# CamilleChallier/Contrastive-Masked-UNet

Hardware: AMD Instinct MI355X
Metric: pretrain images/sec/node at 512x512 (CM-UNet masked-reconstruction step) (higher is better)
Workload: dtype f16; 1 GPU; cmunet_masked_recon_unet64x5_512x512_bs32_mask0.6; optimizer=AdamW(fused), amp=dynamic loss scale (device-side GradScaler protocol), global_batch=32, parallelism=dp1

## Files before the change

### cmunet_amd/_lib.py

```python
import ctypes
import os
import subprocess

_HERE = os.path.dirname(os.path.abspath(__file__))
CSRC = os.path.join(_HERE, "csrc")
LIB_PATH = os.environ.get("CMU_LIB_PATH") or os.path.join(CSRC, "libcmunet_hip.so")

F32, F16, BF16 = 0, 1, 2

_P = ctypes.c_void_p
_I = ctypes.c_int
_L = ctypes.c_int64
_F = ctypes.c_float
_U64 = ctypes.c_uint64
_D = ctypes.c_double

_SIGS = {
    "cmu_last_error": (ctypes.c_char_p, []),
    "cmu_last_kernel": (ctypes.c_char_p, []),
    "cmu_softmax2_threshold": (_I, [_P, _F, _P, _I, _I, _I, _P]),
    "cmu_conv3x3_c1_wgrad_bn": (_I, [_P, _P, _I, _P, _L, _P, _L, _P, _P, _P, _P, _P, _P, _I, _I, _I, _I, _I, _P, _P]),
    "cmu_conv3x3_c1_wgrad_bn_w": (_I, [_P, _P, _I, _P, _L, _P, _P, _P, _P, _P, _P, _P, _I, _I, _I, _I, _I, _P, _P]),
    "cmu_soft_skeleton_ws_bytes": (_L, [_L]),
    "cmu_soft_skeleton": (_I, [_P, _P, _I, _I, _I, _I, _P, _P]),
# ... 37 lines not shown
    "cmu_dtype_size": (_I, [_I]),
    "cmu_pack_conv3x3_elems": (_L, [_I, _I, _I, _I]),
    "cmu_pack_conv3x3": (_I, [_P, _P, _I, _I, _I, _I, _P]),
    "cmu_pack_convT2x2_elems": (_L, [_I, _I, _I, _I]),
    "cmu_pack_convT2x2": (_I, [_P, _P, _I, _I, _I, _I, _P]),
    "cmu_conv3x3_c1_fwd": (_I, [_P, _P, _I, _P, _P, _L, _P, _I, _I, _I, _I, _I, _P]),
    "cmu_conv3x3_fwd": (_I, [_P, _L, _P, _P, _I, _P, _P, _L, _P, _I, _I, _I, _I, _I, _I, _P]),
    "cmu_conv_ntiles": (_I, [_I, _I, _I]),
    "cmu_bn_finalize_ws_bytes": (_L, [_I]),
    "cmu_bn_finalize": (_I, [_P, _I, _L, _P, _P, _P, _P, _P, _F, _F, _I, _P, _P, _P, _P, _I, _P, _P]),
    "cmu_bnrelu_maxpool_fwd": (_I, [_P, _L, _P, _P, _P, _L, _I, _I, _I, _I, _I, _P]),
    "cmu_convT2x2_fwd": (_I, [_P, _L, _P, _P, _I, _P, _P, _P, _L, _I, _I, _I, _I, _I, _I, _P]),
    "cmu_conv1x1_head_fwd": (_I, [_P, _L, _P, _P, _P, _P, _P, _I, _I, _I, _I, _I, _I, _P]),
    "cmu_apply_to_nchw": (_I, [_P, _L, _P, _P, _I, _P, _I, _I, _I, _I, _I, _P]),
    "cmu_nchw_to_nhwc": (_I, [_P, _P, _L, _I, _I, _I, _I, _I, _P]),
    "cmu_nhwc_to_nchw": (_I, [_P, _L, _P, _I, _I, _I, _I, _I, _P]),
    "cmu_bn_bwd_ws_bytes": (_L, [_I]),
    "cmu_bn_bwd_reduce": (_I, [_P, _L, _P, _L, _P, _P, _P, _P, _P, _P, _P, _I, _I, _I, _I, _I, _P, _P]),
    "cmu_bn_bwd_apply": (_I, [_P, _L, _P, _L, _P, _P, _P, _P, _P, _P, _L, _I, _I, _I, _I, _I, _P]),
    "cmu_conv3x3_wgrad_ws_bytes": (_L, [_I, _I, _I, _I, _I, _I]),
    "cmu_conv3x3_wgrad": (_I, [_P, _L, _P, _P, _I, _P, _L, _P, _I, _I, _I, _I, _I, _I, _P, _P]),
    "cmu_conv3x3_c1_wgrad_ws_bytes": (_L, [_I, _I, _I, _I]),
    "cmu_conv3x3_c1_wgrad": (_I, [_P, _P, _I, _P, _L, _P, _I, _I, _I, _I, _I, _P, _P]),
    "cmu_maxpool_bwd": (_I, [_P, _L, _P, _L, _P, _L, _P, _P, _P, _L, _P, _P, _P, _I, _I, _I, _I, _I, _P]),
    "cmu_maxpool_bwd2": (_I, [_P, _L, _P, _L, _P, _L, _P, _L, _P, _P, _P, _L, _P, _P, _P, _I, _I, _I, _I, _I, _P]),
    "cmu_maxpool_bwd_apply": (_I, [_P, _L, _P, _L, _P, _L, _P, _L, _P, _P, _P, _P, _P, _P, _L, _I, _I, _I, _I, _I, _P]),
    "cmu_bnrelu_maxpool_fwd_masked": (_I, [_P, _L, _P, _P, _P, _I, _P, _L, _I, _I, _I, _I, _I, _P]),
    "cmu_maxpool_bwd_masked": (_I, [_P, _L, _P, _L, _P, _L, _P, _P, _P, _I, _P, _L, _I, _I, _I, _I, _I, _P]),
    "cmu_bn_bwd_finalize": (_I, [_P, _L, _P, _P, _P, _I, _P]),
    "cmu_convT2x2_dgrad": (_I, [_P, _L, _P, _P, _L, _I, _I, _I, _I, _I, _I, _P]),
    "cmu_convT2x2_dgrad_bn": (_I, [_P, _L, _P, _P, _L, _P, _L, _P, _P, _P, _P, _P, _I, _I, _I, _I, _I, _I, _P]),
    "cmu_conv3x3_dgrad_bn": (_I, [_P, _L, _P, _P, _L, _P, _L, _P, _P, _P, _P, _P, _I, _I, _I, _I, _I, _I, _P]),
    "cmu_bn_bwd_finalize_tiles": (_I, [_P, _I, _L, _P, _P, _P, _I, _P, _P]),
    "cmu_convT2x2_wgrad_ws_bytes": (_L, [_I, _I, _I, _I, _I, _I]),
    "cmu_convT2x2_wgrad": (_I, [_P, _L, _P, _P, _I, _P, _L, _P, _P, _I, _I, _I, _I, _I, _I, _P, _P]),
    "cmu_conv1x1_head_bwd_ws_bytes": (_L, [_I, _I, _I, _I, _I]),
    "cmu_conv1x1_head_bn_apply": (_I, [_P, _P, _L, _P, _P, _P, _P, _P, _P, _P, _L, _I, _I, _I, _I, _I, _I, _P]),
    "cmu_conv1x1_head_bwd": (_I, [_P, _P, _L, _P, _P, _P, _P, _L, _P, _P, _P, _P, _P, _I, _I, _I, _I, _I, _I, _P, _P]),
    "cmu_masked_mse_ws_bytes": (_L, [_I, _I]),
    "cmu_masked_mse_fwd_bwd": (_I, [_P, _I, _I, _P, _P, _P, _P, _F, _P, _I, _I, _I, _P, _P]),
    "cmu_softmax_ce_dice_ws_bytes": (_L, [_I, _I, _I]),
    "cmu_softmax_ce_dice_fwd_bwd": (_I, [_P, _P, _P, _P, _F, _I, _I, _I, _P, _P]),
    "cmu_infonce_inbatch_fwd_bwd": (_I, [_P, _P, _P, _P, _I, _I, _I, _I, _F, _F, _P]),
    "cmu_moco_ws_bytes": (_L, [_I, _I, _I]),
    "cmu_moco_infonce_enqueue": (_I, [_P, _P, _P, _I, _P, _P, _P, _P, _P, _I, _I, _I, _F, _P, _P]),
    "cmu_l2_normalize_rows": (_I, [_P, _P, _I, _I, _P]),
    "cmu_l2_normalize_rows_bwd": (_I, [_P, _P, _P, _I, _I, _P]),
    "cmu_moco_logits_assemble": (_I, [_P, _P, _P, _P, _I, _I, _I, _F, _P]),
    "cmu_moco_logits_split": (_I, [_P, _P, _I, _I, _F, _P]),
    "cmu_moco_logits_addpos": (_I, [_P, _P, _P, _I, _I, _I, _F, _P]),
    "cmu_row_cross_entropy": (_I, [_P, _P, _P, _P, _P, _P, _I, _I, _P]),
    "cmu_scale_by_device_scalar": (_I, [_P, _P, _L, _P]),
    "cmu_patchify": (_I, [_P, _P, _I, _I, _I, _I, _I, _I, _P]),
    "cmu_masked_stats_rows": (_I, []),
    "cmu_masked_channel_stats": (_I, [_P, _L, _P, _I, _I, _P, _I, _I, _I, _I, _I, _P]),
    "cmu_mask_select": (_I, [_P, _L, _P, _P, _I, _P, _I, _I, _P, _P, _L, _I, _I, _I, _I, _I, _P]),
    "cmu_bn_bwd_reduce_masked": (_I, [_P, _L, _P, _L, _P, _P, _P, _P, _P, _P, _P, _P, _I, _L, _I, _I, _I, _I, _I, _P, _P]),
    "cmu_bn_bwd_apply_masked": (_I, [_P, _L, _P, _L, _P, _P, _P, _P, _P, _P, _L, _P, _I, _I, _I, _I, _I, _I, _P]),
    "cmu_sparse_tile_list": (_I, [_P, _I, _I, _I, _I, _I, _I, _P, _P, _P]),
    "cmu_conv3x3_tiles_supported": (_I, [_I, _I, _I, _I, _I, _I]),
    "cmu_rows_channel_stats": (_I, [_P, _L, _P, _P, _P, _I, _I, _I, _I, _I, _P]),
    "cmu_bn_bwd_reduce_rows": (_I, [_P, _L, _P, _L, _P, _P, _P, _P, _P, _P, _P, _P, _P, _L, _L, _I, _I, _I, _I, _I, _P, _P]),
    "cmu_sparse_tile_lists_max": (_I, []),
    "cmu_sparse_tile_lists": (_I, [_P, _I, _I, _I, _P, _P, _P, _P, _P, _P]),
    "cmu_sparse_pixel_lists": (_I, [_P, _P, _I, _I, _I, _P, _P, _P, _P, _P]),
    "cmu_conv3x3_c1_fwd_tiles_rows": (_I, [_L]),
# ... 191 lines not shown
```

### cmunet_amd/csrc/backward_elem.hip

```cpp
#include "common.h"

constexpr int RED_MAX_BLOCKS = 2048;
#ifndef CMU_POOLB_BLOCKS
#define CMU_POOLB_BLOCKS 2048
#endif
#ifndef CMU_HEADB_BLOCKS
#define CMU_HEADB_BLOCKS 768
#endif
#ifndef CMU_POOLA_PPT
#define CMU_POOLA_PPT 0
#endif
constexpr int POOLB_MAX_BLOCKS = CMU_POOLB_BLOCKS, HEADB_MAX_BLOCKS = CMU_HEADB_BLOCKS;
constexpr int BNWS_HDR = 16;

__device__ static inline float sum_over_rows(float v, float* red, int tid, int cpb, int ppb) {
    __syncthreads();
    red[tid] = v;
    __syncthreads();
    float a = 0.f;
    if (tid < cpb)
        for (int k = 0; k < ppb; ++k) a += red[k * cpb + tid];
    return a;
}

constexpr int FOLD_G = 8;
template <int NV>
__device__ static inline void fold_rows(float (&v)[NV], float* red, int tid, int cpb, int ppb) {
    const int lane = tid & 63, wv = tid >> 6;
    if (cpb <= 64) {
#pragma unroll
        for (int i = 0; i < NV; ++i)
            for (int o = cpb; o < 64; o <<= 1) v[i] += __shfl_xor(v[i], o, 64);
    }
#pragma unroll
    for (int g0 = 0; g0 < NV; g0 += FOLD_G) {
        __syncthreads();
        if (cpb <= 64) {
            if (lane < cpb) {
#pragma unroll
                for (int i = g0; i < g0 + FOLD_G && i < NV; ++i) red[((i - g0) * 4 + wv) * 64 + lane] = v[i];
            }
        } else {
#pragma unroll
            for (int i = g0; i < g0 + FOLD_G && i < NV; ++i) red[(i - g0) * 256 + tid] = v[i];
        }
        __syncthreads();
// ... 66 lines not shown
#pragma unroll
        for (int e = 0; e < EPC; ++e) { t[e] = s1[e]; t[EPC + e] = s2[e]; }
        fold_rows<2 * EPC>(t, red, tid, cpb, ppb);
        if (tid < cpb && blockIdx.y * cpb + tid < nchunk) {
#pragma unroll
            for (int e = 0; e < EPC; ++e) {
                const int c = (blockIdx.y * cpb + tid) * EPC + e;
                ws[((int64_t)blockIdx.x * 2 + 0) * C + c] = t[e];
                ws[((int64_t)blockIdx.x * 2 + 1) * C + c] = t[EPC + e];
            }
        }
        return;
    }
#pragma unroll
    for (int e = 0; e < EPC; ++e) {
        const float a = sum_over_rows(s1[e], red, tid, cpb, ppb);
        const float b = sum_over_rows(s2[e], red, tid, cpb, ppb);
        if (tid < cpb && blockIdx.y * cpb + tid < nchunk) {
            const int c = (blockIdx.y * cpb + tid) * EPC + e;
            ws[((int64_t)blockIdx.x * 2 + 0) * C + c] = a;
            ws[((int64_t)blockIdx.x * 2 + 1) * C + c] = b;
        }
    }
}

__global__ __launch_bounds__(256) void bn_bwd_final_kernel(const float* __restrict__ ws, double count, float* dgamma,
                                                          float* dbeta, float* coef, int C) {
    __shared__ double red[2][16][16];
    const int nblocks = *reinterpret_cast<const int*>(ws);
    ws += BNWS_HDR / 4;
    const int cl = threadIdx.x & 15, part = threadIdx.x >> 4;
    const int c = blockIdx.x * 16 + cl;
    double s1 = 0.0, s2 = 0.0;
    if (c < C) {
        constexpr int U = 8;
        int b = part;
        for (; b + 16 * (U - 1) < nblocks; b += 16 * U) {
            float a[U], q[U];
#pragma unroll
            for (int u = 0; u < U; ++u) {
                a[u] = ws[((int64_t)(b + 16 * u) * 2 + 0) * C + c];
                q[u] = ws[((int64_t)(b + 16 * u) * 2 + 1) * C + c];
            }
#pragma unroll
            for (int u = 0; u < U; ++u) {
                s1 += (double)a[u];
                s2 += (double)q[u];
            }
        }
        for (; b < nblocks; b += 16) {
            s1 += (double)ws[((int64_t)b * 2 + 0) * C + c];
            s2 += (double)ws[((int64_t)b * 2 + 1) * C + c];
        }
    }
    red[0][part][cl] = s1;
    red[1][part][cl] = s2;
    __syncthreads();
    if (part != 0 || c >= C) return;
    s1 = 0.0; s2 = 0.0;
    for (int q = 0; q < 16; ++q) { s1 += red[0][q][cl]; s2 += red[1][q][cl]; }
    if (dbeta) dbeta[c] = (float)s1;
    if (dgamma) dgamma[c] = (float)s2;
    coef[c] = (float)(s1 / count);
    coef[C + c] = (float)(s2 / count);
}

static void chunk_geometry(int nchunk, int* cpb, int* ppb, int* gy) {
    *cpb = nchunk < 256 ? nchunk : 256;
    *ppb = 256 / *cpb;
    *gy = cmu_div_up(nchunk, *cpb);
}

template <class TR>
static int bn_bwd_reduce_t(const void* dA, int64_t ldd, const void* y, int64_t ldy, const float* scale, const float* shift,
                           const float* mean, const float* invstd, float* dgamma, float* dbeta, float* coef, int B, int H, int W,
                           int C, void* ws, const uint8_t* active, int f, int64_t count, hipStream_t st, const int* rows = nullptr,
                           const int* n_rows = nullptr, int64_t max_rows = 0) {
    int cpb, ppb, gy;
    chunk_geometry(C / TR::EPC, &cpb, &ppb, &gy);
    const int64_t npix = (int64_t)B * H * W;
    const int sbits = active ? sp_shift_bits(H, f) : 0;
    const int64_t nloop = rows ? max_rows : npix;
    int gx = (int)(cmu_div_up64(nloop, ppb * 4) < RED_MAX_BLOCKS ? cmu_div_up64(nloop, ppb * 4) : RED_MAX_BLOCKS);
    if (gx < 1) gx = 1;
    hipLaunchKernelGGL((bn_bwd_reduce_kernel<TR>), dim3(gx, gy), dim3(256), 0, st, (const unsigned char*)dA, ldd,
                       (const unsigned char*)y, ldy, scale, shift, mean, invstd, (float*)ws, npix, C, cpb, ppb, active, f, sbits, H, W, rows,
                       n_rows);
// ... 141 lines not shown
}
extern "C" int cmu_bn_bwd_apply(const void* dA, int64_t ldd, const void* y, int64_t ldy, const float* scale, const float* shift,
                                const float* save_mean, const float* save_invstd, const float* coef, void* dY, int64_t ldo, int B,
                                int H, int W, int C, int dt, void* stream) {
    int rc;
    if ((rc = check_pair("cmu_bn_bwd_apply", dA, ldd, y, ldy, C, dt))) return rc;
    if ((rc = check_pair("cmu_bn_bwd_apply(dY)", dY, ldo, y, ldy, C, dt))) return rc;
    CMU_CHECK_ARG(scale && shift && save_mean && save_invstd && coef && B > 0 && H > 0 && W > 0, "cmu_bn_bwd_apply: null argument");
    CMU_DISPATCH_DT(dt, bn_bwd_apply_t, dA, ldd, y, ldy, scale, shift, save_mean, save_invstd, coef, dY, ldo, B, H, W, C,
                    (const uint8_t*)nullptr, 0, (hipStream_t)stream);
}
extern "C" int cmu_bn_bwd_apply_masked(const void* dA, int64_t ldd, const void* y, int64_t ldy, const float* scale, const float* shift,
                                       const float* save_mean, const float* save_invstd, const float* coef, void* dY, int64_t ldo,
                                       const uint8_t* active, int f, int B, int H, int W, int C, int dt, void* stream) {
    int rc;
    if ((rc = check_pair("cmu_bn_bwd_apply_masked", dA, ldd, y, ldy, C, dt))) return rc;
    if ((rc = check_pair("cmu_bn_bwd_apply_masked(dY)", dY, ldo, y, ldy, C, dt))) return rc;
    CMU_CHECK_ARG(scale && shift && save_mean && save_invstd && coef && active && B > 0, "cmu_bn_bwd_apply_masked: null argument");
    CMU_CHECK_ARG(sp_shift_bits(H, f) >= 0 && (f << sp_shift_bits(H, f)) == W, "cmu_bn_bwd_apply_masked: H,W must be f times a power of two");
    CMU_DISPATCH_DT(dt, bn_bwd_apply_t, dA, ldd, y, ldy, scale, shift, save_mean, save_invstd, coef, dY, ldo, B, H, W, C, active, f,
                    (hipStream_t)stream);
}

template <class TR, int MODE>
__global__ __launch_bounds__(256) void maxpool_bwd_kernel(const unsigned char* __restrict__ dP, int64_t ldp,
                                                         const unsigned char* __restrict__ dS, int64_t lds,
                                                         const unsigned char* __restrict__ dS2, int64_t lds2,
                                                         const unsigned char* __restrict__ y, int64_t ldy,
                                                         const float* __restrict__ scale, const float* __restrict__ shift,
                                                         unsigned char* __restrict__ dA, int64_t lda, int B, int H, int W, int C,
                                                         int cpb, int ppb, const float* __restrict__ mean,
                                                         const float* __restrict__ invstd, float* __restrict__ bn_ws,
                                                         const float* __restrict__ coef, const uint8_t* __restrict__ amask = nullptr,
                                                         int mf = 0, int msbits = 0) {
    constexpr int EPC = TR::EPC;
    constexpr int ES = (int)sizeof(typename TR::elem_t);
    __shared__ float red[MODE == 2 ? 1 : FOLD_G * 256];
    const int tid = threadIdx.x;
    const int nchunk = C / EPC;
    const int ch = blockIdx.y * cpb + tid % cpb;
    const int prow = tid / cpb;
    const bool active = prow < ppb && ch < nchunk;
    const int Ho = H / 2, Wo = W / 2;
    const int64_t npool = (int64_t)B * Ho * Wo;
    float sc[EPC], sh[EPC], mu[EPC], is[EPC], s1[EPC], s2[EPC], c1[EPC], c2[EPC];
#pragma unroll
    for (int e = 0; e < EPC; ++e) {
        const int c = active ? ch * EPC + e : 0;
        sc[e] = scale[c];
        sh[e] = shift[c];
        mu[e] = (bn_ws || MODE == 2) ? mean[c] : 0.f;
        is[e] = (bn_ws || MODE == 2) ? invstd[c] : 0.f;
        c1[e] = MODE == 2 ? coef[c] : 0.f;
        c2[e] = MODE == 2 ? coef[C + c] : 0.f;
        s1[e] = s2[e] = 0.f;
    }
    constexpr int PPT = (MODE == 2 && CMU_POOLA_PPT > 0) ? CMU_POOLA_PPT : 0;
    const int64_t span = PPT > 0 ? (int64_t)ppb * PPT : (int64_t)gridDim.x * ppb;
    if (active)
        for (int64_t rng = (int64_t)blockIdx.x * (PPT > 0 ? span : ppb); rng < npool; rng += (PPT > 0 ? (int64_t)gridDim.x * span : npool))
        for (int64_t pp = rng + prow; pp < npool && (PPT == 0 || pp < rng + span); pp += (PPT > 0 ? ppb : span)) {
            int xo, yo, b;
            cmu_pixel_coords(pp, Wo, Ho, npool <= 0x7fffffffll, b, yo, xo);
            if (amask != nullptr && !sp_active(amask, mf, msbits, b, 2 * yo, 2 * xo, 0)) continue;
            float best[EPC], g[EPC], f[4][EPC];
            int arg[EPC];
            TR::unpack(ld_global16_nt(dP + (pp * ldp + ch * EPC) * ES), g);
            int64_t src[4];
#pragma unroll
            for (int q = 0; q < 4; ++q) {
                src[q] = ((int64_t)b * H + 2 * yo + (q >> 1)) * W + 2 * xo + (q & 1);
                TR::unpack(ld_global16(y + (src[q] * ldy + ch * EPC) * ES), f[q]);
#pragma unroll
                for (int e = 0; e < EPC; ++e) {
                    const float a = fmaxf(fmaf(f[q][e], sc[e], sh[e]), 0.f);
// ... 42 lines not shown
        }
    if (MODE == 2 || bn_ws == nullptr) return;
    if (blockIdx.x == 0 && blockIdx.y == 0 && tid == 0) *reinterpret_cast<int*>(bn_ws) = (int)gridDim.x;
    float* ws = bn_ws + BNWS_HDR / 4;
    if (fold_ok(cpb)) {
        float t[2 * EPC];
#pragma unroll
        for (int e = 0; e < EPC; ++e) { t[e] = s1[e]; t[EPC + e] = s2[e]; }
        fold_rows<2 * EPC>(t, red, tid, cpb, ppb);
        if (tid < cpb && blockIdx.y * cpb + tid < nchunk) {
#pragma unroll
            for (int e = 0; e < EPC; ++e) {
                const int c = (blockIdx.y * cpb + tid) * EPC + e;
                ws[((int64_t)blockIdx.x * 2 + 0) * C + c] = t[e];
                ws[((int64_t)blockIdx.x * 2 + 1) * C + c] = t[EPC + e];
            }
        }
        return;
    }
#pragma unroll
    for (int e = 0; e < EPC; ++e) {
        const float a = sum_over_rows(s1[e], red, tid, cpb, ppb);
        const float bsum = sum_over_rows(s2[e], red, tid, cpb, ppb);
        if (tid < cpb && blockIdx.y * cpb + tid < nchunk) {
            const int c = (blockIdx.y * cpb + tid) * EPC + e;
            ws[((int64_t)blockIdx.x * 2 + 0) * C + c] = a;
            ws[((int64_t)blockIdx.x * 2 + 1) * C + c] = bsum;
        }
    }
}
template <class TR>
static int maxpool_bwd_t(const void* dP, int64_t ldp, const void* dS, int64_t lds, const void* dS2, int64_t lds2, const void* y, int64_t ldy, const float* scale,
                         const float* shift, void* dA, int64_t lda, int B, int H, int W, int C, const float* mean, const float* invstd,
                         void* bn_ws, hipStream_t st, const float* coef = nullptr, const uint8_t* amask = nullptr, int mf = 0) {
    int cpb, ppb, gy;
    chunk_geometry(C / TR::EPC, &cpb, &ppb, &gy);
    const int64_t npool = (int64_t)B * (H / 2) * (W / 2);
    int gx = (int)(cmu_div_up64(npool, ppb * 2) < POOLB_MAX_BLOCKS ? cmu_div_up64(npool, ppb * 2) : POOLB_MAX_BLOCKS);
    if (coef != nullptr && CMU_POOLA_PPT > 0) {
        const int64_t nb = cmu_div_up64(npool, (int64_t)ppb * (CMU_POOLA_PPT > 0 ? CMU_POOLA_PPT : 1));
        gx = (int)(nb < (1 << 20) ? nb : (1 << 20));
    }
    if (gx < 1) gx = 1;
#define CMU_POOLB_LAUNCH(MODE_)                                                                                                            \
    hipLaunchKernelGGL((maxpool_bwd_kernel<TR, MODE_>), dim3(gx, gy), dim3(256), 0, st, (const unsigned char*)dP, ldp, (const unsigned char*)dS, lds, \
                       (const unsigned char*)dS2, lds2, (const unsigned char*)y, ldy, scale, shift, (unsigned char*)dA, lda, B, H, W, C, cpb, ppb, \
                       mean, invstd, (float*)bn_ws, coef, amask, mf, amask ? sp_shift_bits(H, mf) : 0)
    if (coef != nullptr) CMU_POOLB_LAUNCH(2);
    else if (dA == nullptr) CMU_POOLB_LAUNCH(1);
    else CMU_POOLB_LAUNCH(0);
#undef CMU_POOLB_LAUNCH
    CMU_CHECK_LAUNCH("cmu_maxpool_bwd");
    return CMU_OK;
}
extern "C" int cmu_maxpool_bwd2(const void* dP, int64_t ldp, const void* dSkip, int64_t lds, const void* dSkip2, int64_t lds2, const void* y,
                                int64_t ldy, const float* scale, const float* shift, void* dA, int64_t lda, const float* save_mean,
                                const float* save_invstd, void* bn_ws, int B, int H, int W, int C, int dt, void* stream) {
    CMU_CHECK_ARG(bn_ws == nullptr || (save_mean && save_invstd), "cmu_maxpool_bwd: fused BN statistics need save_mean / save_invstd");
    CMU_CHECK_ARG(dSkip2 == nullptr || dSkip != nullptr, "cmu_maxpool_bwd2: dSkip2 without dSkip");
    int rc;
    if ((rc = check_pair("cmu_maxpool_bwd(dP,y)", dP, ldp, y, ldy, C, dt))) return rc;
    CMU_CHECK_ARG(dA != nullptr || bn_ws != nullptr, "cmu_maxpool_bwd: dA may only be NULL in the statistics-only form (bn_ws given)");
    if (dA && (rc = check_pair("cmu_maxpool_bwd(dA,y)", dA, lda, y, ldy, C, dt))) return rc;
    if (dSkip && (rc = check_pair("cmu_maxpool_bwd(dSkip,y)", dSkip, lds, y, ldy, C, dt))) return rc;
    if (dSkip2 && (rc = check_pair("cmu_maxpool_bwd2(dSkip2,y)", dSkip2, lds2, y, ldy, C, dt))) return rc;
    CMU_CHECK_ARG(scale && shift && B > 0 && H > 0 && W > 0 && H % 2 == 0 && W % 2 == 0, "cmu_maxpool_bwd: bad dims (%d,%d)", H, W);
    CMU_DISPATCH_DT(dt, maxpool_bwd_t, dP, ldp, dSkip, lds, dSkip2, lds2, y, ldy, scale, shift, dA, lda, B, H, W, C, save_mean, save_invstd,
                    bn_ws, (hipStream_t)stream);
}
extern "C" int cmu_maxpool_bwd_masked(const void* dP, int64_t ldp, const void* dSkip, int64_t lds, const void* y, int64_t ldy, const float* scale,
                                      const float* shift, const uint8_t* active, int f, void* dA, int64_t lda, int B, int H, int W, int C, int dt,
                                      void* stream) {
    CMU_CHECK_ARG(active && f > 0 && dA && scale && shift, "cmu_maxpool_bwd_masked: null argument");
    int rc;
    if ((rc = check_pair("cmu_maxpool_bwd_masked(dP,y)", dP, ldp, y, ldy, C, dt))) return rc;
    if ((rc = check_pair("cmu_maxpool_bwd_masked(dA,y)", dA, lda, y, ldy, C, dt))) return rc;
    if (dSkip && (rc = check_pair("cmu_maxpool_bwd_masked(dSkip,y)", dSkip, lds, y, ldy, C, dt))) return rc;
    CMU_CHECK_ARG(B > 0 && H > 0 && W > 0 && H % 2 == 0 && W % 2 == 0, "cmu_maxpool_bwd_masked: bad dims (%d,%d)", H, W);
    const int sbits = sp_shift_bits(H, f);
    CMU_CHECK_ARG(sbits >= 1 && (f << sbits) == W, "cmu_maxpool_bwd_masked: H=%d, W=%d must be f=%d times a power of two >= 2", H, W, f);
// ... 500 lines not shown
                  "cmu_conv3x3_c1_wgrad_bn: alignment / stride");
    CMU_DISPATCH_DT(dt, conv3x3_c1_wgrad_t, x, mask, mask_per_sample, dA, ldd, dW, B, H, W, Cout, ws, (hipStream_t)stream, yraw, ldy, scale,
                    shift, save_mean, save_invstd, coef);
}
extern "C" int cmu_conv3x3_c1_wgrad_bn_tiles(const float* x, const uint8_t* mask, int mask_per_sample, const void* dA, int64_t ldd,
                                             const void* yraw, int64_t ldy, const float* w, const float* scale, const float* shift,
                                             const float* save_mean, const float* save_invstd, const float* coef, const int* tile_list,
                                             const int* tile_count, int64_t max_tiles, float* dW, int B, int H, int W, int Cout, int dt,
                                             void* ws, void* stream) {
    const int es = cmu_dtype_size(dt);
    CMU_CHECK_ARG(es > 0 && x && dA && scale && shift && save_mean && save_invstd && coef && dW && ws && tile_list && tile_count && B > 0 && H > 0 &&
                      W > 0 && ((yraw != nullptr) != (w != nullptr)),
                  "cmu_conv3x3_c1_wgrad_bn_tiles: bad args (exactly one of yraw / w)");
    const int epc = 16 / es;
    CMU_CHECK_ARG(Cout > 0 && Cout % epc == 0 && Cout / epc <= 256, "cmu_conv3x3_c1_wgrad_bn_tiles: Cout=%d unsupported", Cout);
    CMU_CHECK_ARG(cmu_aligned16(dA) && ldd % epc == 0 && ldd >= Cout && (yraw == nullptr || (cmu_aligned16(yraw) && ldy % epc == 0 && ldy >= Cout)),
                  "cmu_conv3x3_c1_wgrad_bn_tiles: alignment / stride");
    CMU_DISPATCH_DT(dt, conv3x3_c1_wgrad_t, x, mask, mask_per_sample, dA, ldd, dW, B, H, W, Cout, ws, (hipStream_t)stream, yraw, ldy, scale, shift,
                    save_mean, save_invstd, coef, w, tile_list, tile_count, max_tiles);
}
extern "C" int cmu_conv3x3_c1_wgrad_bn_w(const float* x, const uint8_t* mask, int mask_per_sample, const void* dA, int64_t ldd,
                                         const float* w, const float* scale, const float* shift, const float* save_mean,
                                         const float* save_invstd, const float* coef, float* dW, int B, int H, int W, int Cout, int dt,
                                         void* ws, void* stream) {
    const int es = cmu_dtype_size(dt);
    CMU_CHECK_ARG(es > 0 && x && dA && w && scale && shift && save_mean && save_invstd && coef && dW && ws && B > 0 && H > 0 && W > 0,
                  "cmu_conv3x3_c1_wgrad_bn_w: bad args");
    const int epc = 16 / es;
    CMU_CHECK_ARG(Cout > 0 && Cout % epc == 0 && Cout / epc <= 256, "cmu_conv3x3_c1_wgrad_bn_w: Cout=%d unsupported", Cout);
    CMU_CHECK_ARG(cmu_aligned16(dA) && ldd % epc == 0 && ldd >= Cout, "cmu_conv3x3_c1_wgrad_bn_w: alignment / stride");
    CMU_DISPATCH_DT(dt, conv3x3_c1_wgrad_t, x, mask, mask_per_sample, dA, ldd, dW, B, H, W, Cout, ws, (hipStream_t)stream, nullptr, 0, scale,
                    shift, save_mean, save_invstd, coef, w);
}
```

### cmunet_amd/csrc/common.h

```cpp
#pragma once
#include <hip/hip_runtime.h>
#include <stdint.h>
#include <stdio.h>
#include <stdarg.h>
#include "../../include/cmunet_hip.h"

void cmu_set_error(const char* fmt, ...);
void cmu_set_kernel_tag(const char* tag);

#define CMU_CHECK_ARG(cond, ...)                 \
    do {                                         \
        if (!(cond)) {                           \
            cmu_set_error(__VA_ARGS__);          \
            return CMU_ERR_ARG;                  \
        }                                        \
    } while (0)

#define CMU_CHECK_LAUNCH(name)                                                        \
    do {                                                                              \
        hipError_t e__ = hipGetLastError();                                           \
        if (e__ != hipSuccess) {                                                      \
            cmu_set_error("%s: launch failed: %s", name, hipGetErrorString(e__));     \
            return CMU_ERR_LAUNCH;                                                    \
        }                                                                             \
// ... 179 lines not shown
        y = (int)((p / W) % H);
        b = (int)(p / ((int64_t)W * H));
    }
}

__device__ static inline bool sp_active(const uint8_t* __restrict__ active, int f, int sbits, int b, int y, int x, int invert) {
    const bool a = active[((int64_t)b * f + (y >> sbits)) * f + (x >> sbits)] != 0;
    return invert ? !a : a;
}
__host__ __device__ static inline bool cmu_relu_on(int c0, int relu_from) { return relu_from >= 0 ? c0 >= relu_from : c0 < -relu_from; }
static inline int sp_shift_bits(int H, int f) {
    int s = 0;
    while ((f << s) < H) ++s;
    return ((f << s) == H) ? s : -1;
}

constexpr int CMU_TH = 16;
constexpr int CMU_TW = 16;
__host__ __device__ static inline int cmu_div_up(int a, int b) { return (a + b - 1) / b; }
__host__ __device__ static inline int cmu_conv3x3_npad(int N) { return N <= 64 ? 64 : ((N + 127) / 128) * 128; }
static inline int64_t cmu_div_up64(int64_t a, int64_t b) { return (a + b - 1) / b; }

__device__ static inline void philox4x32_10(uint32_t c0, uint32_t c1, uint32_t c2, uint32_t c3, uint32_t k0, uint32_t k1, uint32_t* out) {
#pragma unroll
    for (int r = 0; r < 10; ++r) {
        const uint32_t hi0 = __umulhi(0xD2511F53u, c0), lo0 = 0xD2511F53u * c0;
        const uint32_t hi1 = __umulhi(0xCD9E8D57u, c2), lo1 = 0xCD9E8D57u * c2;
        const uint32_t n0 = hi1 ^ c1 ^ k0, n1 = lo1, n2 = hi0 ^ c3 ^ k1, n3 = lo0;
        c0 = n0; c1 = n1; c2 = n2; c3 = n3;
        k0 += 0x9E3779B9u; k1 += 0xBB67AE85u;
    }
    out[0] = c0; out[1] = c1; out[2] = c2; out[3] = c3;
}
```

### cmunet_amd/csrc/conv_igemm.hip

```cpp
#include "common.h"
#include <stdlib.h>

enum { MODE_CONV3 = 0, MODE_CONVT_FWD = 1, MODE_CONVT_DGRAD = 2 };

struct IGParams {
    const void* x;
    int64_t ldx;
    const float* in_scale;
    const float* in_shift;
    int relu_from;
    const void* w;
    int npad;
    void* y;
    int64_t ldy;
    float* stats;
    const float* bias;
    int B, H, W;
    int K;
    int N;
    int Cq;
    int nslices;
    int nslices32;
    int tilesX, tilesY, nblk;
    int64_t total_blocks;
    const void* bx;
    int64_t ldbx;
    const float *b_scale, *b_shift, *b_mean, *b_invstd;
    float* bstats;
    int buf_ok;
    unsigned fd_nblk[2], fd_tx[2], fd_ty[2];
    const int* tile_list;
    const int* tile_count;
};
static inline void cmu_fastdiv_init(unsigned d, unsigned* out) {
    unsigned s = 0;
    while ((1ull << s) < d) ++s;
    out[0] = (unsigned)((((1ull << s) - d) << 32) / d + 1);
    out[1] = s;
}

template <class TR, int MODE>
struct IGCfg {
    typedef typename TR::elem_t elem_t;
    static constexpr bool C3 = (MODE == MODE_CONV3);
    static constexpr int TAPS = C3 ? 9 : 2;
    static constexpr int HALO = C3 ? 1 : 0;
    static constexpr int LW = CMU_TW + 2 * HALO;
    static constexpr int LH = CMU_TH + 2 * HALO;
    static constexpr int NPIX = LW * LH;
    static constexpr int SLICES_A = C3 ? 1 : TAPS;
    static constexpr int PS_A = SLICES_A * 64 + 16;
    static constexpr int A_BYTES = NPIX * PS_A;
    static constexpr int PS_W = 80;
    static constexpr int BN = 64;
    static constexpr int W_BYTES = TAPS * BN * PS_W;
    static constexpr int KC = 64 / (int)sizeof(elem_t);
    static constexpr int EPC = TR::EPC;
    static constexpr int EPI_ROW = BN * (int)sizeof(elem_t) + 16;
    static constexpr int EPI_STAGE = 4 * 64 * EPI_ROW;
    static constexpr int EPI_BYTES = EPI_STAGE + 4 * BN * 2 * 4;
    static constexpr int MAIN_BYTES = A_BYTES + W_BYTES;
    static constexpr int LDS_BYTES = MAIN_BYTES > EPI_BYTES ? MAIN_BYTES : EPI_BYTES;
    static constexpr int A_CHUNKS = NPIX * SLICES_A * 4;
    static constexpr int A_ITERS = (A_CHUNKS + 255) / 256;
    static constexpr int W_CHUNKS = TAPS * BN * 4;
    static constexpr int W_ITERS = (W_CHUNKS + 255) / 256;
// ... 263 lines not shown
        IG_STAMP(5);
    }
    __syncthreads();

    float* stat_lds = reinterpret_cast<float*>(smem + C::EPI_STAGE);
    if (MODE == MODE_CONV3 && p.stats != nullptr) {
        float s1[2] = {0.f, 0.f}, s2[2] = {0.f, 0.f};
#pragma unroll
        for (int i = 0; i < 2; ++i)
#pragma unroll
            for (int e = 0; e < 16; ++e) {
                const int m32 = (e & 3) + 8 * (e >> 2) + 4 * h;
                const int row = 4 * wave + 2 * i + pm_row(m32), col = pm_col(m32);
                const bool ok = (ty0 + row < p.H) && (tx0 + col < p.W);
#pragma unroll
                for (int j = 0; j < 2; ++j) {
                    const float v = ok ? acc[i][j][e] : 0.f;
                    s1[j] += v;
                    s2[j] = fmaf(v, v, s2[j]);
                }
            }
#pragma unroll
        for (int j = 0; j < 2; ++j) {
            s1[j] += __shfl_xor(s1[j], 32, 64);
            s2[j] += __shfl_xor(s2[j], 32, 64);
            if (h == 0) {
                stat_lds[(wave * C::BN + 32 * j + r) * 2 + 0] = s1[j];
                stat_lds[(wave * C::BN + 32 * j + r) * 2 + 1] = s2[j];
            }
        }
    }
    constexpr int CPRp = C::BN / C::EPC;
    u32x4 xr[CPRp];
    if ((MODE != MODE_CONVT_FWD) && p.bstats != nullptr) {
#pragma unroll
        for (int it = 0; it < CPRp; ++it) {
            const int idx = it * 64 + lane;
            const int m = idx / CPRp, q = idx % CPRp;
            const int row = 4 * wave + 2 * (m >> 5) + pm_row(m & 31), col = pm_col(m & 31);
            const int gy = ty0 + row < p.H ? ty0 + row : p.H - 1, gx = tx0 + col < p.W ? tx0 + col : p.W - 1;
            int n = n0 + q * C::EPC;
            n = n < p.N ? n : 0;
            const int64_t xo = (((int64_t)b * p.H + gy) * p.W + gx) * p.ldbx + n;
            xr[it] = ld_global16(reinterpret_cast<const unsigned char*>(p.bx) + xo * (int64_t)sizeof(elem_t));
        }
    }
    unsigned char* my = smem + wave * (64 * C::EPI_ROW);
#pragma unroll
    for (int i = 0; i < 2; ++i)
#pragma unroll
        for (int j = 0; j < 2; ++j) {
            float badd = 0.f;
            if (MODE == MODE_CONVT_FWD) {
                const int n = n0 + 32 * j + r;
                if (n < p.N) badd = p.bias[n % p.Cq];
            }
#pragma unroll
            for (int e = 0; e < 16; ++e) {
                const int m = 32 * i + (e & 3) + 8 * (e >> 2) + 4 * h;
                *reinterpret_cast<elem_t*>(my + m * C::EPI_ROW + (32 * j + r) * (int)sizeof(elem_t)) =
                    TR::from_float(acc[i][j][e] + badd);
            }
        }
    __syncthreads();
    if (MODE == MODE_CONV3 && p.stats != nullptr && tid < C::BN) {
        const int n = n0 + tid;
        if (n < p.N) {
            float a = 0.f, q = 0.f;
#pragma unroll
            for (int w4 = 0; w4 < 4; ++w4) {
                a += stat_lds[(w4 * C::BN + tid) * 2 + 0];
                q += stat_lds[(w4 * C::BN + tid) * 2 + 1];
            }
            p.stats[(tile * 2 + 0) * p.N + n] = a;
            p.stats[(tile * 2 + 1) * p.N + n] = q;
        }
    }
    constexpr int CPR = C::BN / C::EPC;
    unsigned char* yb = reinterpret_cast<unsigned char*>(p.y);
    const bool bs = (MODE != MODE_CONVT_FWD) && p.bstats != nullptr;
    constexpr int EPCc = C::EPC;
    float bsc[EPCc], bsh[EPCc], bmu[EPCc], bis[EPCc], bs1[EPCc], bs2[EPCc];
    const int nq = n0 + (lane % CPR) * EPCc;
    if (bs) {
#pragma unroll
        for (int e = 0; e < EPCc; ++e) {
            const int c = nq + e < p.N ? nq + e : 0;
            bsc[e] = p.b_scale[c]; bsh[e] = p.b_shift[c]; bmu[e] = p.b_mean[c]; bis[e] = p.b_invstd[c];
            bs1[e] = bs2[e] = 0.f;
        }
    }
#pragma unroll
    for (int it = 0; it < (64 * CPR) / 64; ++it) {
        const int idx = it * 64 + lane;
        const int m = idx / CPR, q = idx % CPR;
        const int row = 4 * wave + 2 * (m >> 5) + pm_row(m & 31), col = pm_col(m & 31);
        const int gy = ty0 + row, gx = tx0 + col;
        const int n = n0 + q * C::EPC;
        if (gy < p.H && gx < p.W && n < p.N) {
            const u32x4 v = *reinterpret_cast<const u32x4*>(my + m * C::EPI_ROW + q * 16);
            int64_t off;
            if (MODE == MODE_CONVT_FWD) {
                const int ij = n / p.Cq, co = n % p.Cq;
                off = (((int64_t)b * (2 * p.H) + 2 * gy + (ij >> 1)) * (2 * p.W) + 2 * gx + (ij & 1)) * p.ldy + co;
            } else {
                off = (((int64_t)b * p.H + gy) * p.W + gx) * p.ldy + n;
            }
            st_global16(yb + off * (int64_t)sizeof(elem_t), v);
            if (bs) {
                float gv[EPCc], xv[EPCc];
                TR::unpack(v, gv);
                TR::unpack(xr[it], xv);
#pragma unroll
                for (int e = 0; e < EPCc; ++e) {
                    const float dz = fmaf(xv[e], bsc[e], bsh[e]) > 0.f ? gv[e] : 0.f;
                    bs1[e] += dz;
                    bs2[e] = fmaf(dz, xv[e], bs2[e]);
                }
            }
        }
    }
    if (bs) {
#pragma unroll
        for (int e = 0; e < EPCc; ++e) {
#pragma unroll
            for (int o = CPR; o < 64; o <<= 1) {
                bs1[e] += __shfl_xor(bs1[e], o, 64);
                bs2[e] += __shfl_xor(bs2[e], o, 64);
            }
            bs2[e] = (bs2[e] - bmu[e] * bs1[e]) * bis[e];
            if (lane < CPR) {
                stat_lds[(wave * C::BN + lane * EPCc + e) * 2 + 0] = bs1[e];
                stat_lds[(wave * C::BN + lane * EPCc + e) * 2 + 1] = bs2[e];
            }
        }
        __syncthreads();
        if (tid < C::BN && n0 + tid < p.N) {
            float a = 0.f, q = 0.f;
#pragma unroll
            for (int w4 = 0; w4 < 4; ++w4) {
                a += stat_lds[(w4 * C::BN + tid) * 2 + 0];
                q += stat_lds[(w4 * C::BN + tid) * 2 + 1];
            }
            p.bstats[(tile * 2 + 0) * p.N + n0 + tid] = a;
            p.bstats[(tile * 2 + 1) * p.N + n0 + tid] = q;
        }
    }
}

#include "conv_igemm3.inc"
#include "conv_igemm3p.inc"
#include "conv_igemm5.inc"
#include "conv_igemm6.inc"
#include "conv_gemm.inc"
#include "conv_gather.inc"

template <class TR, int MODE>
static int launch_igemm(const IGParams& p, hipStream_t st, const char* name) {
    typedef IGCfg<TR, MODE> C;
    static CmuPerDevice attr_set;
    if (!attr_set.done()) {
        hipError_t e = hipFuncSetAttribute(reinterpret_cast<const void*>(&conv_igemm_kernel<TR, MODE>),
                                           hipFuncAttributeMaxDynamicSharedMemorySize, C::LDS_BYTES);
        if (e != hipSuccess) {
            cmu_set_error("%s: hipFuncSetAttribute(%d B LDS): %s", name, C::LDS_BYTES, hipGetErrorString(e));
            return CMU_ERR_LAUNCH;
        }
        attr_set.mark();
    }
    hipLaunchKernelGGL((conv_igemm_kernel<TR, MODE>), dim3((unsigned)p.total_blocks), dim3(256), C::LDS_BYTES, st, p);
    cmu_set_kernel_tag("conv_igemm_kernel");
    CMU_CHECK_LAUNCH(name);
    return CMU_OK;
}

static int check_act(const char* name, const void* ptr, int64_t ld, int C, int dt) {
    const int epc = 16 / cmu_dtype_size(dt);
    CMU_CHECK_ARG(ptr != nullptr, "%s: null tensor", name);
// ... 343 lines not shown
    for (int i = 0; i < n; ++i) {
        const int sb = sp_shift_bits(H[i], f);
        CMU_CHECK_ARG(rows[i] && counts[i] && capacity[i] > 0 && sb >= 0 && (int64_t)B * H[i] * H[i] < (1ll << 31),
                      "cmu_sparse_pixel_lists: null list, or H must be f << s (entry %d: H=%d, f=%d)", i, H[i], f);
        q.s[i] = 1 << sb; q.H[i] = H[i]; q.rows[i] = rows[i]; q.count[i] = counts[i]; q.cap[i] = capacity[i];
        if (capacity[i] > cmax) cmax = capacity[i];
    }
    const int grid = (int)(cmu_div_up64(cmax, 256) < 4096 ? cmu_div_up64(cmax, 256) : 4096);
    hipLaunchKernelGGL(sparse_pixel_rows_multi_kernel, dim3(grid, n), dim3(256), 0, (hipStream_t)stream, patches, patch_count, q);
    CMU_CHECK_LAUNCH("cmu_sparse_pixel_lists");
    return CMU_OK;
}
extern "C" int cmu_sparse_tile_list(const uint8_t* active, int f, int B, int H, int W, int tile_h, int tile_w, int* list, int* count,
                                    void* stream) {
    CMU_CHECK_ARG(active && list && count && f > 0 && B > 0 && H > 0 && W > 0 && tile_h > 0 && tile_w > 0, "cmu_sparse_tile_list: bad args");
    const int sbits = sp_shift_bits(H, f);
    CMU_CHECK_ARG(sbits >= 0 && W == H, "cmu_sparse_tile_list: H must be f << s and the level square (H=%d, W=%d, f=%d)", H, W, f);
    const int tilesY = cmu_div_up(H, tile_h), tilesX = cmu_div_up(W, tile_w);
    CMU_CHECK_ARG((int64_t)B * tilesY * tilesX < (1ll << 30), "cmu_sparse_tile_list: too many tiles");
    hipLaunchKernelGGL(sparse_tile_list_kernel, dim3(1), dim3(1024), 0, (hipStream_t)stream, active, f, sbits, B, tilesY, tilesX, tile_h, tile_w,
                       list, count);
    CMU_CHECK_LAUNCH("cmu_sparse_tile_list");
    return CMU_OK;
}

static int check_bnstats(const char* name, const void* yraw, int64_t ldy, const float* scale, const float* shift, const float* mean,
                         const float* invstd, const float* bstats, int N, int dt) {
    int rc;
    if ((rc = check_act(name, yraw, ldy, N, dt))) return rc;
    CMU_CHECK_ARG(scale && shift && mean && invstd && bstats, "%s: null BatchNorm argument", name);
    return CMU_OK;
}

extern "C" int cmu_conv3x3_dgrad_bn(const void* dY, int64_t ldd, const void* wpacked_flip, void* dX, int64_t ldx, const void* yraw,
                                    int64_t ldy, const float* scale, const float* shift, const float* save_mean,
                                    const float* save_invstd, float* bstats, int B, int H, int W, int K, int N, int dt, void* stream) {
    CMU_CHECK_ARG(B > 0 && H > 0 && W > 0 && K > 0 && N > 0, "cmu_conv3x3_dgrad_bn: bad dims");
    CMU_CHECK_ARG(cmu_dtype_size(dt) > 0, "cmu_conv3x3_dgrad_bn: bad dtype %d", dt);
    int rc;
    if ((rc = check_act("cmu_conv3x3_dgrad_bn(dY)", dY, ldd, K, dt))) return rc;
    if ((rc = check_act("cmu_conv3x3_dgrad_bn(dX)", dX, ldx, N, dt))) return rc;
    if ((rc = check_bnstats("cmu_conv3x3_dgrad_bn(yraw)", yraw, ldy, scale, shift, save_mean, save_invstd, bstats, N, dt))) return rc;
    CMU_CHECK_ARG(wpacked_flip && cmu_aligned16(wpacked_flip), "cmu_conv3x3_dgrad_bn: packed weights null/unaligned");
    CMU_CHECK_ARG((int64_t)B * cmu_div_up(H, CMU_TH) * cmu_div_up(W, CMU_TW) * cmu_div_up(N, 64) < (1ll << 31), "cmu_conv3x3_dgrad_bn: grid too large");
    IGParams p = {};
    p.x = dY; p.ldx = ldd; p.w = wpacked_flip; p.y = dX; p.ldy = ldx;
    p.B = B; p.H = H; p.W = W; p.K = K; p.N = N; p.Cq = N;
    p.bx = yraw; p.ldbx = ldy; p.b_scale = scale; p.b_shift = shift; p.b_mean = save_mean; p.b_invstd = save_invstd; p.bstats = bstats;
    fill_tiles(p);
    CMU_DISPATCH_DT(dt, conv3x3_fwd_t, p, (hipStream_t)stream);
}

extern "C" int cmu_convT2x2_dgrad_bn(const void* dOut, int64_t ldd, const void* wpacked_dgrad, void* dX, int64_t ldx, const void* yraw,
                                     int64_t ldy, const float* scale, const float* shift, const float* save_mean,
                                     const float* save_invstd, float* bstats, int B, int H, int W, int Cin, int Cout, int dt,
                                     void* stream) {
    CMU_CHECK_ARG(B > 0 && H > 0 && W > 0 && Cin > 0 && Cout > 0, "cmu_convT2x2_dgrad_bn: bad dims");
    CMU_CHECK_ARG(cmu_dtype_size(dt) > 0, "cmu_convT2x2_dgrad_bn: bad dtype %d", dt);
    int rc;
    if ((rc = check_act("cmu_convT2x2_dgrad_bn(dOut)", dOut, ldd, Cout, dt))) return rc;
    if ((rc = check_act("cmu_convT2x2_dgrad_bn(dX)", dX, ldx, Cin, dt))) return rc;
    if ((rc = check_bnstats("cmu_convT2x2_dgrad_bn(yraw)", yraw, ldy, scale, shift, save_mean, save_invstd, bstats, Cin, dt))) return rc;
    CMU_CHECK_ARG(wpacked_dgrad && cmu_aligned16(wpacked_dgrad), "cmu_convT2x2_dgrad_bn: packed weights null/unaligned");
    IGParams p = {};
    p.x = dOut; p.ldx = ldd; p.w = wpacked_dgrad; p.y = dX; p.ldy = ldx;
    p.B = B; p.H = H; p.W = W; p.K = Cout; p.N = Cin; p.Cq = Cout;
    p.bx = yraw; p.ldbx = ldy; p.b_scale = scale; p.b_shift = shift; p.b_mean = save_mean; p.b_invstd = save_invstd; p.bstats = bstats;
    fill_tiles(p);
    CMU_DISPATCH_DT(dt, convT_dgrad_t, p, (hipStream_t)stream);
}
```

### cmunet_amd/csrc/conv_igemm3.inc

```
#include <type_traits>

template <class TR, int NB_, int TWB_ = 2, int THB_ = 1>
struct IG3Cfg {
    typedef typename TR::elem_t elem_t;
    static constexpr int ES = (int)sizeof(elem_t);
    static constexpr int EPC = TR::EPC;
    static constexpr int KC = 32 / ES;
    static constexpr int NB = NB_;
    static constexpr int TWB = TWB_;
    static constexpr int THB = THB_;
    static constexpr int TH = 16 * THB, TW = 16 * TWB;
    static constexpr int LW = TW + 2, LH = TH + 2, NPIX = LW * LH;
    static constexpr int PS = 48;
    static constexpr int A_BYTES = NPIX * PS;
    static constexpr int PSB = 32;
    static constexpr int B_TAP = NB * PSB;
    static constexpr int B_BYTES = 9 * B_TAP;
    static constexpr int BUF_BYTES = A_BYTES + B_BYTES;
    static constexpr int MAIN_BYTES = 2 * BUF_BYTES;
    static constexpr int WN = NB / 64, WM = 8 / WN;
    static constexpr int RB = WM / TWB;
    static constexpr int SW = TH / 2 / RB;
    static constexpr int A_CHUNKS = NPIX * 2, A_ITERS = (A_CHUNKS + 511) / 512;
    static constexpr int B_CHUNKS = 9 * NB * 2, B_ITERS = (B_CHUNKS + 511) / 512;
// ... 94 lines not shown
    }
}

template <class TR, int NB, int TWB>
__device__ __forceinline__ void ig3_epilogue(const IGParams& p, unsigned char* smem, f32x16 (&acc)[IG3Cfg<TR, NB, TWB>::SW][2], int tid, int lane,
                                             int wave, int wn, int wrow, int wcol, int r, int h, int b, int ty, int tx, int ty0, int tx0,
                                             int n0) {
    typedef IG3Cfg<TR, NB, TWB> C;
    typedef typename TR::elem_t elem_t;
    constexpr int EPC = TR::EPC;
    constexpr int SW = C::SW;
    float* stat_lds = reinterpret_cast<float*>(smem + C::EPI_STAGE);
    const int row0 = wrow * 2 * SW, col0 = wcol * 16;
    if (p.stats != nullptr) {
        float s1[2], s2[2];
        ig3_lane_stats<SW>(acc, [&](int i, int e) {
            const int m32 = (e & 3) + 8 * (e >> 2) + 4 * h;
            const int row = row0 + 2 * i + pm_row(m32), col = col0 + pm_col(m32);
            return (ty0 + row < p.H) && (tx0 + col < p.W);
        }, s1, s2);
#pragma unroll
        for (int j = 0; j < 2; ++j) {
            s1[j] += __shfl_xor(s1[j], 32, 64);
            s2[j] += __shfl_xor(s2[j], 32, 64);
            if (h == 0) {
                stat_lds[(wave * 64 + 32 * j + r) * 2 + 0] = s1[j];
                stat_lds[(wave * 64 + 32 * j + r) * 2 + 1] = s2[j];
            }
        }
    }
    unsigned char* my = smem + wave * C::EPI_WAVE;
    unsigned char* yb = reinterpret_cast<unsigned char*>(p.y);
    constexpr int CPR = C::NFP * 32 / EPC;
    auto write_slab = [&](float* dst) {
        if (tid < TWB * NB) {
            const int half = tid / NB, c = tid % NB;
            const int tx16 = TWB * tx + half, tiles16 = (p.W + 15) / 16;
            if (tx16 < tiles16 && n0 + c < p.N) {
                float a = 0.f, q = 0.f;
#pragma unroll
                for (int wr = 0; wr < C::RB; ++wr) {
                    const int wv = (c / 64) * C::WM + wr * TWB + half;
                    a += stat_lds[(wv * 64 + (c & 63)) * 2 + 0];
                    q += stat_lds[(wv * 64 + (c & 63)) * 2 + 1];
                }
                const int64_t t16 = ((int64_t)b * p.tilesY + ty) * tiles16 + tx16;
                dst[(t16 * 2 + 0) * p.N + n0 + c] = a;
                dst[(t16 * 2 + 1) * p.N + n0 + c] = q;
            }
        }
    };
    constexpr int NIT = (SW * 32 * CPR) / 64;
    float badd[2] = {0.f, 0.f};
    const bool cq64 = p.bias != nullptr && (p.Cq & 63) == 0;
    int ij_w = 0, co_w = 0;
    if (p.bias != nullptr) {
        const int nw = n0 + wn * 64;
        ij_w = nw / p.Cq;
        co_w = nw - ij_w * p.Cq;
#pragma unroll
        for (int j = 0; j < 2; ++j) badd[j] = p.bias[cq64 ? co_w + 32 * j + r : (nw + 32 * j + r) % p.Cq];
    }
#pragma unroll
    for (int jp = 0; jp < 2 / C::NFP; ++jp) {
        if (jp > 0) __syncthreads();
        u32x4 xr[NIT];
        if (p.bstats != nullptr) {
#pragma unroll
            for (int it = 0; it < NIT; ++it) {
                const int idx = it * 64 + lane;
                const int m = idx / CPR, q = idx % CPR;
                const int row = row0 + 2 * (m >> 5) + pm_row(m & 31), col = col0 + pm_col(m & 31);
                const int gy = ty0 + row < p.H ? ty0 + row : p.H - 1, gx = tx0 + col < p.W ? tx0 + col : p.W - 1;
                const int n = n0 + wn * 64 + jp * C::NFP * 32 + q * EPC;
                const int64_t pixel = ((int64_t)b * p.H + gy) * p.W + gx;
                xr[it] = ld_global16(reinterpret_cast<const unsigned char*>(p.bx) + (pixel * p.ldbx + n) * (int64_t)sizeof(elem_t));
            }
        }
#pragma unroll
        for (int i = 0; i < SW; ++i)
#pragma unroll
            for (int jj = 0; jj < C::NFP; ++jj)
#pragma unroll
                for (int e = 0; e < 16; ++e) {
                    const int m = 32 * i + (e & 3) + 8 * (e >> 2) + 4 * h;
                    *reinterpret_cast<elem_t*>(my + m * C::EPI_ROW + (32 * jj + r) * C::ES) =
                        TR::from_float(acc[i][jp * C::NFP + jj][e] + badd[jp * C::NFP + jj]);
                }
        __syncthreads();
        if (jp == 0 && p.stats != nullptr) write_slab(p.stats);
        float bsc[EPC], bsh[EPC], bs1[EPC], bs2[EPC];
        const int nq = n0 + wn * 64 + jp * C::NFP * 32 + (lane % CPR) * EPC;
        if (p.bstats != nullptr) {
            ig3_bst_consts<EPC>(p.b_scale, p.b_shift, nq, bsc, bsh);
#pragma unroll
            for (int e = 0; e < EPC; ++e) bs1[e] = bs2[e] = 0.f;
        }
#pragma unroll
        for (int it = 0; it < NIT; ++it) {
            const int idx = it * 64 + lane;
            const int m = idx / CPR, q = idx % CPR;
            const int row = row0 + 2 * (m >> 5) + pm_row(m & 31), col = col0 + pm_col(m & 31);
            const int gy = ty0 + row, gx = tx0 + col;
            const int n = n0 + wn * 64 + jp * C::NFP * 32 + q * EPC;
            if (gy < p.H && gx < p.W) {
                const u32x4 v = *reinterpret_cast<const u32x4*>(my + m * C::EPI_ROW + q * 16);
                const int64_t pixel = ((int64_t)b * p.H + gy) * p.W + gx;
                if (p.bias != nullptr) {
                    const int ij = cq64 ? ij_w : n / p.Cq, co = cq64 ? co_w + (n - (n0 + wn * 64)) : n % p.Cq;
                    const int64_t po = ((int64_t)b * (2 * p.H) + 2 * gy + (ij >> 1)) * (2 * p.W) + 2 * gx + (ij & 1);
                    st_global16_nt(yb + (po * p.ldy + co) * (int64_t)sizeof(elem_t), v);
                } else {
                    st_global16_nt(yb + (pixel * p.ldy + n) * (int64_t)sizeof(elem_t), v);
                }
                if (p.bstats != nullptr) ig3_bst_accum<TR>(v, xr[it], bsc, bsh, bs1, bs2);
            }
        }
        if (p.bstats != nullptr) {
            const int nb0 = n0 + wn * 64 + jp * C::NFP * 32;
            ig3_bst_fold<EPC>(bs1, bs2, lane, p.b_mean + nb0, p.b_invstd + nb0, stat_lds + (wave * 64 + jp * C::NFP * 32) * 2);
        }
    }
    if (p.bstats != nullptr) {
        __syncthreads();
        write_slab(p.bstats);
    }
}

template <class TR, int NB, bool TF, int TWB>
__global__ __launch_bounds__(512) void conv_igemm3_kernel(const IGParams p) {
    typedef IG3Cfg<TR, NB, TWB> C;
    constexpr int EPC = TR::EPC;
    constexpr int SW = C::SW;
    extern __shared__ __attribute__((aligned(16))) unsigned char smem[];

    const int tid = threadIdx.x;
    const int lane = tid & 63;
    const int wave = __builtin_amdgcn_readfirstlane(tid >> 6);
    const int r = lane & 31;
    const int h = lane >> 5;
    const int wm = wave % C::WM, wn = wave / C::WM;
    const int wcol = wm % TWB, wrow = wm / TWB;

    int64_t bid = blockIdx.x;
    {
        const int64_t nb = p.total_blocks;
        const int64_t q = nb >> 3, rem = nb & 7;
        const int64_t xcd = bid & 7, local = bid >> 3;
        bid = (xcd < rem ? xcd * (q + 1) : rem * (q + 1) + (xcd - rem) * q) + local;
    }
    const int nbk = (int)(bid % p.nblk);
    const int64_t tile = bid / p.nblk;
    const int tx = (int)(tile % p.tilesX);
    const int ty = (int)((tile / p.tilesX) % p.tilesY);
    const int b = (int)(tile / ((int64_t)p.tilesX * p.tilesY));
    const int ty0 = ty * C::TH, tx0 = tx * C::TW;
    const int n0 = nbk * NB;

// ... 278 lines not shown
```

### cmunet_amd/csrc/conv_igemm3p.inc

```

template <class TR, int NB, int THB = 1, bool WRES = false>
struct IG3PCfg {
    typedef IG3Cfg<TR, NB, 2, THB> C;
    static constexpr int WRES_SLICES = 4;
    static constexpr int A_STRIDE = WRES ? C::A_BYTES : C::BUF_BYTES;
    static constexpr int B_BASE = WRES ? 2 * C::A_BYTES : C::A_BYTES;
    static constexpr int MAIN_BYTES = WRES ? 2 * C::A_BYTES + WRES_SLICES * C::B_BYTES : C::MAIN_BYTES;
    static constexpr int STAT_OFF = MAIN_BYTES + C::TAB_BYTES;
    static constexpr int STAT_BYTES = 8 * 64 * 2 * 4;
    static constexpr int EPI_OFF = STAT_OFF + STAT_BYTES;
    static constexpr int EPI_WAVE1 = 16 * C::EPI_ROW;
#ifdef CMU_IG_STAMPS
    static constexpr int STAMP_OFF = MAIN_BYTES + 1024;
    static constexpr int STAMP_ITERS = 12;
    static constexpr int LDS_BYTES = EPI_OFF + 8 * EPI_WAVE1;
#else
    static constexpr int LDS_BYTES = EPI_OFF + 8 * EPI_WAVE1;
#endif
};

template <class TR, int NB, bool TF, bool BST, int THB = 1, bool WRES = false, bool PART = false>
__global__ __launch_bounds__(512) void conv_igemm3p_kernel(const IGParams p) {
    typedef IG3Cfg<TR, NB, 2, THB> C;
    typedef IG3PCfg<TR, NB, THB, WRES> P;
// ... 238 lines not shown
        constexpr bool FULL = decltype(full_c)::value;
        const int ty0 = t.ty * C::TH, tx0 = t.tx * C::TW;
        unsigned char* yb = reinterpret_cast<unsigned char*>(p.y);
        int lane = tid & 63;
        asm volatile("" : "+v"(lane));
        const int r = lane & 31, h = lane >> 5;
        unsigned char* my = smem + P::EPI_OFF + (wave & 3) * (2 * P::EPI_WAVE1);
        if (!BST && p.stats != nullptr) {
            float s1[2], s2[2];
            if constexpr (FULL) {
                ig3_lane_stats<SW>(acc, [](int, int) { return true; }, s1, s2);
            } else {
                ig3_lane_stats<SW>(acc, [&](int i, int e) {
                    const int m32 = (e & 3) + 8 * (e >> 2) + 4 * h;
                    return (ty0 + row0 + 2 * i + pm_row(m32) < p.H) && (tx0 + col0 + pm_col(m32) < p.W);
                }, s1, s2);
            }
            IG3P_STAMP_E(7);
#pragma unroll
            for (int j = 0; j < 2; ++j) {
                s1[j] += __shfl_xor(s1[j], 32, 64);
                s2[j] += __shfl_xor(s2[j], 32, 64);
                const int ch = ILV ? 2 * r + j : 32 * j + r;
                if (h == 0) {
                    stat_lds[(wave * 64 + ch) * 2 + 0] = s1[j];
                    stat_lds[(wave * 64 + ch) * 2 + 1] = s2[j];
                }
            }
        }
        IG3P_STAMP_E(4);
        const int q = lane % CPR;
        const int64_t pix0 = ((int64_t)t.b * p.H + ty0 + row0) * p.W + tx0 + col0;
        const int cl = (lane >> 3) & 3;
        unsigned yoff[2], xoff[2];
#pragma unroll
        for (int c = 0; c < 2; ++c) {
            yoff[c] = (unsigned)((((h ^ c) * p.W + cl) * p.ldy + q * EPC) * C::ES);
            xoff[c] = BST ? (unsigned)((((h ^ c) * p.W + cl) * p.ldbx + q * EPC) * C::ES) : 0u;
        }
#pragma unroll
        for (int jp = 0; jp < 2 / C::NFP; ++jp) {
            const int n = t.n0 + wn * 64 + jp * C::NFP * 32 + q * EPC;
            const int nw = t.n0 + wn * 64 + jp * C::NFP * 32;
            unsigned char* ybase = yb + (pix0 * p.ldy + nw) * (int64_t)C::ES;
            const unsigned char* xbase = reinterpret_cast<const unsigned char*>(p.bx) + (pix0 * p.ldbx + nw) * (int64_t)C::ES;
            float bsc[EPC], bsh[EPC], bs1[EPC], bs2[EPC];
            if (BST) {
                ig3_bst_consts<EPC>(p.b_scale, p.b_shift, n, bsc, bsh);
#pragma unroll
                for (int e = 0; e < EPC; ++e) bs1[e] = bs2[e] = 0.f;
            }
            auto load_x = [&](int u, u32x4* xr) {
#pragma unroll
                for (int it = 0; it < NIT; ++it) {
                    if (FULL) {
                        const int soff = ((2 * (u >> 1)) * p.W + 4 * (2 * (u & 1) + it)) * (int)p.ldbx * C::ES;
                        xr[it] = ld_global16(xbase + soff + xoff[(it ^ u) & 1]);
                    } else {
                        const int m = 16 * (u & 1) + (it * 64 + lane) / CPR;
                        const int row = row0 + 2 * (u >> 1) + pm_row(m), col = col0 + pm_col(m);
                        const int gy = ty0 + row < p.H ? ty0 + row : p.H - 1, gx = tx0 + col < p.W ? tx0 + col : p.W - 1;
                        const int64_t pixel = ((int64_t)t.b * p.H + gy) * p.W + gx;
                        xr[it] = ld_global16(reinterpret_cast<const unsigned char*>(p.bx) + (pixel * p.ldbx + n) * (int64_t)sizeof(elem_t));
                    }
                }
            };
            auto write_unit = [&](int u) {
                const int i = u >> 1, hs = u & 1;
                unsigned char* st = my + (u & 1) * P::EPI_WAVE1;
                if constexpr (ILV) {
                    static_assert(C::NFP == 2, "both n-fragments of a 16-bit tile are staged in one pass");
#pragma unroll
                    for (int e = 0; e < 8; ++e) {
                        const int ml = (e & 3) + 8 * (e >> 2) + 4 * h;
                        *reinterpret_cast<uint32_t*>(st + ml * C::EPI_ROW + r * 4) = TR::pack2(acc[i][0][8 * hs + e], acc[i][1][8 * hs + e]);
                    }
                } else
#pragma unroll
                for (int jj = 0; jj < C::NFP; ++jj)
#pragma unroll
                    for (int e8 = 0; e8 < 8; e8 += 2) {
                        const int ml = (e8 & 3) + 8 * (e8 >> 2) + 4 * h;
                        const float va = acc[i][jp * C::NFP + jj][8 * hs + e8], vb = acc[i][jp * C::NFP + jj][8 * hs + e8 + 1];
                        unsigned char* d0 = st + ml * C::EPI_ROW + (32 * jj + r) * C::ES;
                        if constexpr (sizeof(elem_t) == 2) {
                            const uint32_t pk = TR::pack2(va, vb);
                            *reinterpret_cast<uint16_t*>(d0) = (uint16_t)pk;
                            *reinterpret_cast<uint16_t*>(d0 + C::EPI_ROW) = (uint16_t)(pk >> 16);
                        } else {
                            *reinterpret_cast<elem_t*>(d0) = TR::from_float(va);
                            *reinterpret_cast<elem_t*>(d0 + C::EPI_ROW) = TR::from_float(vb);
                        }
                    }
            };
            u32x4 xr[2][NIT];
            if (BST) load_x(0, xr[0]);
            write_unit(0);
#pragma unroll
            for (int u = 0; u < 2 * SW; ++u) {
                const int i = u >> 1, hs = u & 1;
                if (BST && u + 1 < 2 * SW) load_x(u + 1, xr[(u + 1) & 1]);
                __builtin_amdgcn_wave_barrier();
                u32x4 v[NIT];
#pragma unroll
                for (int it = 0; it < NIT; ++it) {
                    const int ml = (it * 64 + lane) / CPR;
                    v[it] = *reinterpret_cast<const u32x4*>(my + (u & 1) * P::EPI_WAVE1 + ml * C::EPI_ROW + q * 16);
                }
                __builtin_amdgcn_sched_barrier(0);
                if (u + 1 < 2 * SW) write_unit(u + 1);
                __builtin_amdgcn_sched_barrier(0);
#pragma unroll
                for (int it = 0; it < NIT; ++it) {
                    const int soff = ((2 * i) * p.W + 4 * (2 * hs + it)) * (int)p.ldy * C::ES;
                    bool inimg = true;
                    if constexpr (!FULL)
                        inimg = (ty0 + row0 + 2 * i + (h ^ ((it ^ hs) & 1)) < p.H) && (tx0 + col0 + 4 * (2 * hs + it) + cl < p.W);
                    if (inimg) {
                        st_global16_nt(ybase + soff + yoff[(it ^ hs) & 1], v[it]);
                        if (BST) ig3_bst_accum<TR>(v[it], xr[u & 1][it], bsc, bsh, bs1, bs2);
                    }
                }
                if (u == SW - 1) IG3P_STAMP_E(5);
            }
            IG3P_STAMP_E(6);
            __builtin_amdgcn_wave_barrier();
            if (BST) ig3_bst_fold<EPC>(bs1, bs2, lane, p.b_mean + nw, p.b_invstd + nw, stat_lds + (wave * 64 + jp * C::NFP * 32) * 2);
        }
    };
    auto epilogue = [&](const Item t) { epilogue_impl(t, std::integral_constant<bool, !PART>{}); };
    auto write_slab = [&](const Item t) {
        float* dst = BST ? p.bstats : p.stats;
        int tid = threadIdx.x;
        asm volatile("" : "+v"(tid));
        if (dst != nullptr && tid < TWB * THB * NB) {
            const int blk = tid / NB, c = tid % NB;
            const int vhalf = blk / TWB, half = blk % TWB;
            const int tx16 = TWB * t.tx + half, tiles16 = (p.W + 15) / 16;
            if (tx16 < tiles16 && t.n0 + c < p.N) {
                float a = 0.f, q2 = 0.f;
#pragma unroll
                for (int wr = 0; wr < C::RB / THB; ++wr) {
                    const int wv = (c / 64) * C::WM + (vhalf * (C::RB / THB) + wr) * TWB + half;
                    a += stat_lds[(wv * 64 + (c & 63)) * 2 + 0];
                    q2 += stat_lds[(wv * 64 + (c & 63)) * 2 + 1];
                }
                const int64_t t16 = ((int64_t)t.b * (THB * p.tilesY) + THB * t.ty + vhalf) * tiles16 + tx16;
                dst[(t16 * 2 + 0) * p.N + t.n0 + c] = a;
                dst[(t16 * 2 + 1) * p.N + t.n0 + c] = q2;
            }
        }
    };

    if (WRES) {
#pragma unroll
        for (int s = 0; s < P::WRES_SLICES; ++s) {
            u32x4 wr[C::B_ITERS];
#pragma unroll
            for (int it = 0; it < C::B_ITERS; ++it)
                wr[it] = ig3_bload(rs_w, it < C::B_ITERS - 1 ? b_voff0 : b_voff_last, (unsigned)s * w_slice + it * b_it_bytes);
#pragma unroll
            for (int it = 0; it < C::B_ITERS; ++it)
                if (it < C::B_ITERS - 1 || b_last_live) *reinterpret_cast<u32x4*>(smem + s * C::B_BYTES + b_st + it * (256 * C::PSB)) = wr[it];
        }
    }
    set_load_tile(0);
    issue_loads();
    {
        u32x4 a0[C::A_ITERS], b0[C::B_ITERS];
#pragma unroll
        for (int it = 0; it < C::A_ITERS; ++it) a0[it] = areg[it];
        if (!WRES) {
#pragma unroll
            for (int it = 0; it < C::B_ITERS; ++it) b0[it] = breg[it];
        }
        advance();
        issue_loads();
        __syncthreads();
        u32x4 a1[C::A_ITERS], b1[C::B_ITERS];
#pragma unroll
        for (int it = 0; it < C::A_ITERS; ++it) { a1[it] = areg[it]; areg[it] = a0[it]; }
        if (!WRES) {
// ... 179 lines not shown
```

### cmunet_amd/csrc/conv_igemm5.inc

```
#ifndef CMU_V5_ST_NT
#define CMU_V5_ST_NT 1
#endif
struct IG5Cfg {
    static constexpr int ES = 2, EPC = 8;
    static constexpr int KC = 32;
    static constexpr int NB = 128;
    static constexpr int TH = 16, TW = 32, LW = TW + 2, LH = TH + 2, NPIX = LW * LH;
    static constexpr int PLANE = NPIX * 32;
    static constexpr int PSTRIDE = PLANE + 64;
    static constexpr int A_BYTES = 2 * PSTRIDE;
    static constexpr int MAIN_BYTES = 2 * A_BYTES;
    static constexpr int MAX_K = 1024;
    static constexpr int TAB_BYTES = 2 * MAX_K * 4;
    static constexpr int STAT_OFF = MAIN_BYTES + TAB_BYTES;
    static constexpr int STAT_PAR = 8 * 64 * 2 * 4;
    static constexpr int BX_OFF = STAT_OFF + 2 * STAT_PAR;
    static constexpr int BX_WAVE = 8 * 1024, BX_BYTES = 8 * BX_WAVE;
    static constexpr int STAMP_OFF = BX_OFF + BX_BYTES;
    static constexpr int STAMP_ITERS = 16;
#ifdef CMU_IG_STAMPS
    static constexpr int LDS_BYTES = STAMP_OFF + 2 * STAMP_ITERS * 8 * 8;
    static constexpr int LDS_BYTES_BST = LDS_BYTES;
#else
    static constexpr int LDS_BYTES = STAT_OFF + 2 * STAT_PAR;
// ... 380 lines not shown
                        }
                        sv[2 * (4 * j + e)] = s1;
                        sv[2 * (4 * j + e) + 1] = s2;
                    }
                ig5_row16_sum_batch(sv);
                if (n16 == 0) {
#pragma unroll
                    for (int j = 0; j < 4; ++j) {
                        float* d = stat_lds + (32 * (j >> 1) + 8 * g + 4 * (j & 1)) * 2;
                        *reinterpret_cast<f32x4*>(d) = f32x4{sv[8 * j], sv[8 * j + 1], sv[8 * j + 2], sv[8 * j + 3]};
                        *reinterpret_cast<f32x4*>(d + 4) = f32x4{sv[8 * j + 4], sv[8 * j + 5], sv[8 * j + 6], sv[8 * j + 7]};
                    }
                }
            }
#ifdef CMU_IG_STAMPS_EPI
            IG5_STAMP(1);
#endif
#pragma unroll
            for (int i = 0; i < EROWS; ++i) {
                u32x4 v[2];
#pragma unroll
                for (int s = 0; s < 2; ++s) {
                    v[s][0] = TR::pack2(acc[i][2 * s][0], acc[i][2 * s][1]);
                    v[s][1] = TR::pack2(acc[i][2 * s][2], acc[i][2 * s][3]);
                    v[s][2] = TR::pack2(acc[i][2 * s + 1][0], acc[i][2 * s + 1][1]);
                    v[s][3] = TR::pack2(acc[i][2 * s + 1][2], acc[i][2 * s + 1][3]);
                }
                ig5_store_row_lines(ybase + i * yrow, offA, offB, lo, v[0], v[1]);
            }
#ifdef CMU_IG_STAMPS_EPI
            IG5_STAMP(2);
#endif
        } else {
            const unsigned char* xbase = reinterpret_cast<const unsigned char*>(p.bx) + (pix0 * p.ldbx + nw) * (int64_t)C::ES;
            const unsigned xoff = (unsigned)((pi * (int)p.ldbx + 8 * g) * C::ES);
            const int64_t xrow = (int64_t)p.W * p.ldbx * C::ES;
            float bsc[2][EPC], bsh[2][EPC], bs1[2][EPC], bs2[2][EPC];
#pragma unroll
            for (int s = 0; s < 2; ++s) {
                ig3_bst_consts<EPC>(p.b_scale, p.b_shift, nw + 32 * s + 8 * g, bsc[s], bsh[s]);
#pragma unroll
                for (int e = 0; e < EPC; ++e) bs1[s][e] = bs2[s][e] = 0.f;
            }
#ifdef CMU_IG_STAMPS_EPI
            IG5_STAMP(1);
#endif
            const unsigned char* bxl = smem + C::BX_OFF + wave * C::BX_WAVE + (ln & 63) * 16;
            u32x4 xr[2][2];
#pragma unroll
            for (int s = 0; s < 2; ++s) xr[0][s] = ld_global16(xbase + 4 * xrow + s * 64 + xoff);
#pragma unroll
            for (int i = 0; i < 8; ++i) {
                if (i < 4) {
#pragma unroll
                    for (int s = 0; s < 2; ++s) xr[1][s] = *reinterpret_cast<const u32x4*>(bxl + (i * 2 + s) * 1024);
                } else if (i + 1 < 8) {
#pragma unroll
                    for (int s = 0; s < 2; ++s) xr[(i + 1) & 1][s] = ld_global16(xbase + (i + 1) * xrow + s * 64 + xoff);
                }
                u32x4 v[2];
#pragma unroll
                for (int s = 0; s < 2; ++s) {
                    v[s][0] = TR::pack2(acc[i][2 * s][0], acc[i][2 * s][1]);
                    v[s][1] = TR::pack2(acc[i][2 * s][2], acc[i][2 * s][3]);
                    v[s][2] = TR::pack2(acc[i][2 * s + 1][0], acc[i][2 * s + 1][1]);
                    v[s][3] = TR::pack2(acc[i][2 * s + 1][2], acc[i][2 * s + 1][3]);
                    ig3_bst_accum<TR>(v[s], xr[i < 4 ? 1 : (i & 1)][s], bsc[s], bsh[s], bs1[s], bs2[s]);
                }
                ig5_store_row_lines(ybase + i * yrow, offA, offB, lo, v[0], v[1]);
            }
#ifdef CMU_IG_STAMPS_EPI
            IG5_STAMP(2);
#endif
            float sv[32];
#pragma unroll
            for (int s = 0; s < 2; ++s)
#pragma unroll
                for (int e = 0; e < EPC; ++e) {
                    sv[2 * (8 * s + e)] = bs1[s][e];
                    sv[2 * (8 * s + e) + 1] = bs2[s][e];
                }
            ig5_row16_sum_batch(sv);
            if (n16 == 0) {
#pragma unroll
                for (int s = 0; s < 2; ++s) {
                    float* d = stat_lds + (32 * s + 8 * g) * 2;
#pragma unroll
                    for (int q = 0; q < 4; ++q) *reinterpret_cast<f32x4*>(d + 4 * q) = f32x4{sv[16 * s + 4 * q], sv[16 * s + 4 * q + 1], sv[16 * s + 4 * q + 2], sv[16 * s + 4 * q + 3]};
                }
            }
        }
    };
    auto write_slab = [&](const Item t, int par) {
        float* dst = BST ? p.bstats : p.stats;
        int tl = threadIdx.x;
        asm volatile("" : "+v"(tl));
        if (dst != nullptr && tl < 2 * C::NB) {
            const float* stat_lds = reinterpret_cast<const float*>(smem + C::STAT_OFF + par * C::STAT_PAR);
            const int half = tl / C::NB, c = tl % C::NB;
            const int tx16 = 2 * t.tx + half, tiles16 = p.W / 16;
            float a = 0.f, q2 = 0.f;
#pragma unroll
            for (int wr = 0; wr < 2; ++wr) {
                const int wv = (c / 64) * 4 + wr * 2 + half;
                a += stat_lds[(wv * 64 + (c & 63)) * 2 + 0];
                q2 += stat_lds[(wv * 64 + (c & 63)) * 2 + 1];
            }
            if (BST) q2 = (q2 - p.b_mean[t.n0 + c] * a) * p.b_invstd[t.n0 + c];
            const int64_t t16 = ((int64_t)t.b * p.tilesY + t.ty) * tiles16 + tx16;
            dst[(t16 * 2 + 0) * p.N + t.n0 + c] = a;
            dst[(t16 * 2 + 1) * p.N + t.n0 + c] = q2;
        }
    };

    set_load_tile(0);
    int n0_mma = decode_n0(0);
    issue_loads();
    {
        u32x4 a0[C::A_ITERS];
#pragma unroll
        for (int it = 0; it < C::A_ITERS; ++it) a0[it] = areg[it];
        advance();
        issue_loads();
        __syncthreads();
        u32x4 a1[C::A_ITERS];
#pragma unroll
        for (int it = 0; it < C::A_ITERS; ++it) { a1[it] = areg[it]; areg[it] = a0[it]; }
        s_regs = 0;
        inb_regs = a_inb;
        store_regs();
#pragma unroll
        for (int it = 0; it < C::A_ITERS; ++it) areg[it] = a1[it];
        s_regs = s_ld;
    }
    __builtin_amdgcn_s_waitcnt(0x0f70);
    __syncthreads();
    load_w(w0, (unsigned)(n0_mma + wn * 64) * 32u);

    const int second = wave >= 4 ? 1 : 0;
    if (second && 1 < G) stage_phase();
    else issue_loads_stream();
    int s_mma = 0, i_mma = 0, epi_ops = 0;
#pragma unroll 1
    for (int g = 0; g < G; ++g) {
        const unsigned soff_cur = (unsigned)s_mma * w_s64 + (unsigned)(n0_mma + wn * 64) * 32u;
        int n0_next = n0_mma;
        unsigned soff_next;
        if (s_mma + 1 < nsl) soff_next = soff_cur + w_s64;
        else {
            if (i_mma + 1 < n_my) n0_next = decode_n0(i_mma + 1);
            soff_next = (unsigned)(n0_next + wn * 64) * 32u;
        }
        const bool last = s_mma == nsl - 1;
#ifdef CMU_IG_STAMPS
        stamp_g = g;
#endif
        IG5_STAMP(0);
        auto issue_bx_dma = [&]() {
            if constexpr (BST) {
                const Item t = decode(i_mma);
                const int64_t pix0 = ((int64_t)t.b * p.H + t.ty * C::TH + 8 * wrow) * p.W + t.tx * C::TW + 16 * wcol;
                const uint64_t xa = reinterpret_cast<uint64_t>(p.bx) + (uint64_t)((pix0 * p.ldbx + t.n0 + wn * 64) * (int64_t)C::ES);
                typedef __attribute__((ext_vector_type(4))) int i32x4_t;
                const i32x4_t xd = {__builtin_amdgcn_readfirstlane((int)(uint32_t)xa), __builtin_amdgcn_readfirstlane((int)((xa >> 32) & 0xffffu)), -1, 0x00020000};
                int ln = tid & 63;
                asm volatile("" : "+v"(ln));
                const int n16l = ln & 15, gl = ln >> 4;
                const int pil = n16l < 4 ? n16l : (n16l < 12 ? n16l + 4 : n16l - 8);
                const unsigned xoffl = (unsigned)((pil * (int)p.ldbx + 8 * gl) * C::ES);
                const unsigned xrowl = (unsigned)((int64_t)p.W * p.ldbx * C::ES);
                const unsigned lds0 = (unsigned)(C::BX_OFF + wave * C::BX_WAVE);
#pragma unroll
                for (int i = 0; i < 4; ++i)
#pragma unroll
                    for (int s = 0; s < 2; ++s) {
                        const unsigned m0v = (unsigned)__builtin_amdgcn_readfirstlane((int)(lds0 + (i * 2 + s) * 1024));
                        const unsigned so = (unsigned)__builtin_amdgcn_readfirstlane((int)(i * xrowl + s * 64));
                        asm volatile("s_mov_b32 m0, %0\n\ts_nop 0\n\tbuffer_load_dwordx4 %1, %2, %3 offen lds" :: "s"(m0v), "v"(xoffl), "s"(xd), "s"(so) : "memory", "m0");
                    }
            }
        };
        if (BST && last) issue_bx_dma();
        __builtin_amdgcn_s_setprio(2);
        mfma_step((unsigned)(g & 1) * C::A_BYTES, soff_cur, soff_next, epi_ops, BST && last);
        __builtin_amdgcn_s_setprio(0);
        IG5_STAMP(3);
        if (second) __syncthreads();
        IG5_STAMP(4);
        const bool staging = g + second + 1 < G;
        IG5_WAIT_VM(4);
        if (staging) store_regs();
        if (s_mma == 1 && i_mma > 0) write_slab(decode(i_mma - 1), (i_mma - 1) & 1);
        if (staging) advance();
        if (!BST) issue_loads_stream();
        IG5_STAMP(5);
        epi_ops = 0;
        if (last) {
            epilogue(decode(i_mma), i_mma & 1);
            zero_acc();
#ifdef CMU_V5_MOCK_WINO
            epi_ops = 4;
#else
            epi_ops = BST ? 24 : 16;
// ... 30 lines not shown
    static_assert(C::LDS_BYTES <= 163840 && C::LDS_BYTES_BST <= 163840, "LDS budget");
    static CmuPerDevice attr_set;
    if (!attr_set.done()) {
        hipError_t e = hipFuncSetAttribute(reinterpret_cast<const void*>(&conv_igemm5_kernel<TR, TF, BST>),
                                           hipFuncAttributeMaxDynamicSharedMemorySize, BST ? C::LDS_BYTES_BST : C::LDS_BYTES);
        if (e != hipSuccess) {
            cmu_set_error("cmu_conv3x3_fwd(16x16x32, persistent): hipFuncSetAttribute(%d B LDS): %s", C::LDS_BYTES, hipGetErrorString(e));
            return CMU_ERR_LAUNCH;
        }
        attr_set.mark();
    }
    p.tilesX = p.W / C::TW;
    p.tilesY = p.H / C::TH;
    p.nblk = p.N / C::NB;
    p.nslices = p.K / C::KC;
    p.nslices32 = p.K / 16;
    p.npad = cmu_conv3x3_npad(p.N);
    p.total_blocks = (int64_t)p.B * p.tilesX * p.tilesY * p.nblk;
#ifdef CMU_V5_MOCK_WINO
    p.total_blocks *= 4;
#endif
    cmu_fastdiv_init((unsigned)p.nblk, p.fd_nblk);
    cmu_fastdiv_init((unsigned)p.tilesX, p.fd_tx);
    cmu_fastdiv_init((unsigned)p.tilesY, p.fd_ty);
    static const int forced = []() { const char* e = getenv("CMU_CONV_PERSIST_GRID"); return e ? atoi(e) : 0; }();
    const int64_t want = forced > 0 ? forced : cmu_num_cus();
    const int64_t grid = p.total_blocks < want ? p.total_blocks : want;
    hipLaunchKernelGGL((conv_igemm5_kernel<TR, TF, BST>), dim3((unsigned)grid), dim3(512), BST ? C::LDS_BYTES_BST : C::LDS_BYTES, st, p);
    cmu_set_kernel_tag("conv_igemm5_kernel");
    CMU_CHECK_LAUNCH("cmu_conv3x3_fwd(16x16x32, persistent)");
    return CMU_OK;
}

template <class TR>
static bool igemm5_eligible(const IGParams& p) {
    if constexpr (sizeof(typename TR::elem_t) != 2) return false;
    if (!cmu_switch_on(CMU_SW_CONV_V5)) return false;
    if (p.tile_list != nullptr) return false;
    if (p.in_scale != nullptr && p.bstats != nullptr) return false;
    if (p.N % 128 != 0 || p.K % 64 != 0) return false;
    static const int min_k = []() { const char* e = getenv("CMU_V5_MIN_K"); return e ? atoi(e) : 128; }();
    static const int min_k_bst = []() { const char* e = getenv("CMU_V5_MIN_K_BST"); return e ? atoi(e) : 256; }();
    if (p.K < min_k || (p.bstats != nullptr && p.K < min_k_bst)) return false;
    if (p.H % 16 != 0 || p.W % 32 != 0) return false;
    if ((int64_t)p.B * (p.H / 16) * (p.W / 32) * (p.N / 128) >= (1ll << 30)) return false;
    return !igemm3_narrow_blocks(p);
}
template <class TR>
static int launch_igemm5(const IGParams& p, hipStream_t st) {
    if constexpr (sizeof(typename TR::elem_t) == 2) {
        const bool tf = p.in_scale != nullptr, bst = p.bstats != nullptr;
        return tf ? launch_igemm5_cfg<TR, true, false>(p, st) : (bst ? launch_igemm5_cfg<TR, false, true>(p, st) : launch_igemm5_cfg<TR, false, false>(p, st));
    } else {
        return CMU_ERR_ARG;
    }
}
```

### cmunet_amd/csrc/elementwise.hip

```cpp
#include "common.h"
#include <string.h>

static thread_local char g_err[512] = "";
void cmu_set_error(const char* fmt, ...) {
    va_list ap;
    va_start(ap, fmt);
    vsnprintf(g_err, sizeof(g_err), fmt, ap);
    va_end(ap);
}
extern "C" const char* cmu_last_error(void) { return g_err; }
static thread_local const char* g_kernel_tag = "";
void cmu_set_kernel_tag(const char* tag) { g_kernel_tag = tag; }
extern "C" const char* cmu_last_kernel(void) { return g_kernel_tag; }
extern "C" int cmu_version(void) { return 100; }

static const char* const g_switch_names[CMU_SW_COUNT] = {"CMU_CONV_NARROW", "CMU_CONV_SLIM", "CMU_CONV_PERSIST_PART", "CMU_WGRAD_SQUARE",
                                                         "CMU_WGRAD_WIDE_F32", "CMU_CONV_V5", "CMU_CONV_V6"};
static int g_switch_env[CMU_SW_COUNT] = {-1, -1, -1, -1, -1, -1, -1};
static int g_switch_override[CMU_SW_COUNT] = {-1, -1, -1, -1, -1, -1, -1};
bool cmu_switch_on(int id) {
    const int ov = __atomic_load_n(&g_switch_override[id], __ATOMIC_RELAXED);
    if (ov >= 0) return ov != 0;
    int v = __atomic_load_n(&g_switch_env[id], __ATOMIC_RELAXED);
    if (v < 0) {
// ... 322 lines not shown
    const int c = blockIdx.x * 16 + cl;
    double s1 = 0.0, s2 = 0.0;
    if (c < C)
        for (int s = part; s < nsplit; s += 16) {
            s1 += ws[((int64_t)s * 2 + 0) * C + c];
            s2 += ws[((int64_t)s * 2 + 1) * C + c];
        }
    red[0][part][cl] = s1;
    red[1][part][cl] = s2;
    __syncthreads();
    if (part != 0 || c >= C) return;
    s1 = 0.0; s2 = 0.0;
    for (int q = 0; q < 16; ++q) { s1 += red[0][q][cl]; s2 += red[1][q][cl]; }
    if (dbeta) dbeta[c] = (float)s1;
    if (dgamma) dgamma[c] = (float)s2;
    coef[c] = (float)(s1 / count);
    coef[C + c] = (float)(s2 / count);
}
extern "C" int cmu_bn_bwd_finalize_tiles(const float* bstats, int ntiles, int64_t count, float* dgamma, float* dbeta, float* coef, int C,
                                         void* ws, void* stream) {
    CMU_CHECK_ARG(bstats && coef && ws && C > 0 && ntiles > 0 && count > 0, "cmu_bn_bwd_finalize_tiles: bad args");
    hipStream_t st = (hipStream_t)stream;
    int nsplit = ntiles / 16;
    if (nsplit < 1) nsplit = 1;
    if (nsplit > BN_MAX_SPLITS) nsplit = BN_MAX_SPLITS;
    hipLaunchKernelGGL(bn_reduce_slab_kernel, dim3(cmu_div_up(C, 64), nsplit), dim3(256), 0, st, bstats, ntiles, C, nsplit, (double*)ws);
    CMU_CHECK_LAUNCH("cmu_bn_bwd_finalize_tiles(reduce)");
    hipLaunchKernelGGL(bn_bwd_final_tiles_kernel, dim3(cmu_div_up(C, 16)), dim3(256), 0, st, (const double*)ws, nsplit, (double)count,
                       dgamma, dbeta, coef, C);
    CMU_CHECK_LAUNCH("cmu_bn_bwd_finalize_tiles");
    return CMU_OK;
}

#ifndef CMU_C1F_WAVES
#define CMU_C1F_WAVES 4
#endif
template <class TR>
__global__ __launch_bounds__(256, CMU_C1F_WAVES) void conv3x3_c1_fwd_kernel(const float* __restrict__ x, const uint8_t* __restrict__ mask,
                                                            int mask_per_sample, const float* __restrict__ w,
                                                            typename TR::elem_t* __restrict__ y, int64_t ldy, float* stats, int B,
                                                            int H, int W, int Cout, int tilesX, int tilesY,
                                                            const int* __restrict__ tlist = nullptr, const int* __restrict__ tcount = nullptr) {
    constexpr int EPC = TR::EPC;
    __shared__ float halo[2][18 * 18];
    __shared__ float red[2][256];
    const int tid = threadIdx.x;
    const int nchunk = Cout / EPC;
    const int ppi = 256 / nchunk;
    const int chunk = tid % nchunk, prow = tid / nchunk;
    const bool active = prow < ppi;
    float wr[EPC][9];
#pragma unroll
    for (int e = 0; e < EPC; ++e)
#pragma unroll
        for (int t = 0; t < 9; ++t) wr[e][t] = active ? w[(chunk * EPC + e) * 9 + t] : 0.f;
    const int ntile = B * tilesX * tilesY;
    const int tpi = tilesX * tilesY;
    float hv[2];
    auto halo_load = [&](int tile) {
        const int tx = tile % tilesX, ty = (tile / tilesX) % tilesY, b = tile / tpi;
#pragma unroll
        for (int k = 0; k < 2; ++k) {
            const int i = tid + k * 256;
            const int gy = ty * 16 - 1 + i / 18, gx = tx * 16 - 1 + i % 18;
            float v = 0.f;
            if (i < 18 * 18 && gy >= 0 && gy < H && gx >= 0 && gx < W) {
// ... 371 lines not shown
```

### cmunet_amd/engine.py

```python
import os
import weakref

import torch

from . import _lib, ops
from .ops import Act
from .optim import claim_grad_sink

BN_EPS = 1e-5
BN_MOMENTUM = 0.1


_FUSE_HEAD = os.environ.get("CMU_HEAD_FUSE", "1") != "0"
_FUSE_DGRAD_BN = os.environ.get("CMU_DGRAD_BN", "1")
_FUSE_POOL = os.environ.get("CMU_POOL_FUSE", "1") != "0"
_POISON_NEW = os.environ.get("CMU_POISON_NEW", "0") == "1"
_FUSE_POOL2 = os.environ.get("CMU_POOL_FUSE2", "1") != "0"
_C1W_RECOMP = os.environ.get("CMU_C1W_RECOMP", "1") != "0"


class _Scratch:

    def __init__(self, device):
        self.device = device
        self.bufs = {}

    def get(self, key, nbytes):
        nbytes = max(int(nbytes), 16)
        b = self.bufs.get(key)
        if b is None or b.numel() < nbytes:
            b = torch.empty(nbytes, dtype=torch.uint8, device=self.device)
            self.bufs[key] = b
        return b


class _PackCache:

    def __init__(self):
        self.items = {}

    def get(self, key, param, fn):
        ver = (param._version, ops.PARAM_GENERATION)
        hit = self.items.get(key)
        if hit is not None and hit[0] == ver and hit[1] == param.data_ptr():
            return hit[2]
        packed = fn()
        self.items[key] = (ver, param.data_ptr(), packed)
        return packed


class _Ctx(dict):
# ... 86 lines not shown
        stats = ops.new_stats(B, H, W, Cout, self.device) if training else None
        if x_img is not None:
            ops.conv3x3_c1_fwd(x_img, w.detach(), out, stats, mask, mask_per_sample)
        else:
            ops.conv3x3_fwd(x, self._wp(pconv, w, False), out, stats)
        scale, shift = affine_out if affine_out is not None else (self._f32(Cout), self._f32(Cout))
        mean, invstd = self._f32(Cout), self._f32(Cout)
        ws = self.scratch.get("bnfin", self.lib.cmu_bn_finalize_ws_bytes(Cout))
        ops.bn_finalize(stats, B * H * W, sd[pconv + "bias"].detach(), sd[pbn + "weight"].detach(),
                        sd[pbn + "bias"].detach(), sd[pbn + "running_mean"], sd[pbn + "running_var"], BN_MOMENTUM,
                        BN_EPS, training, scale, shift, mean, invstd, ws)
        if training and (pbn + "num_batches_tracked") in sd:
            self._nbt.append(sd[pbn + "num_batches_tracked"])
        return {"pconv": pconv, "pbn": pbn, "x": x, "x_img": x_img, "mask": mask, "mps": mask_per_sample,
                "y": out.with_transform(scale, shift, 0), "mean": mean, "invstd": invstd,
                "w_ver": (w._version, w.data_ptr(), ops.PARAM_GENERATION) if x_img is not None else None}

    def _double_conv_fwd(self, sd, prefix, x, out2, training, x_img=None, mask=None, mask_per_sample=False, affine_out2=None):
        w1 = sd[prefix + "0.weight"]
        B, H, W = out2.B, out2.H, out2.W
        y1 = self._new(B, H, W, w1.shape[0])
        s1 = self._convbn_fwd(sd, prefix + "0.", prefix + "1.", x, y1, training, x_img, mask, mask_per_sample)
        s2 = self._convbn_fwd(sd, prefix + "3.", prefix + "4.", s1["y"], out2, training, affine_out=affine_out2)
        self.flush_counters()
        return s1, s2

    def _bn_ws(self, C):
        return self.scratch.get("bnbwd", self.lib.cmu_bn_bwd_ws_bytes(C))

    def _tile_slab(self, y):
        n = ops.ntiles(y.B, y.H, y.W)
        return self.scratch.get("bst", n * 2 * y.C * 4)[:n * 2 * y.C * 4].view(torch.float32).view(n, 2, y.C)

    def _convbn_bwd(self, sd, s, dA, grads, need_dx, dx_out=None, fused_stats=False, next_bn=None, head=None, pool=None):
        y = s["y"]
        B, H, W, C = y.B, y.H, y.W, y.C
        w = sd[s["pconv"] + "weight"]
        dgamma, dbeta = self._gbuf(s["pbn"] + "weight", sd[s["pbn"] + "weight"]), self._gbuf(s["pbn"] + "bias", sd[s["pbn"] + "bias"])
        coef = self._f32(2, C)
        ws = self._bn_ws(C)
        bst = s.pop("bstats", None)
        if bst is not None:
            ops.bn_bwd_finalize_tiles(bst, B * H * W, dgamma, dbeta, coef,
                                      self.scratch.get("bnfin", self.lib.cmu_bn_finalize_ws_bytes(C)))
        elif fused_stats:
            ops.bn_bwd_finalize(ws, B * H * W, dgamma, dbeta, coef)
        else:
            ops.bn_bwd_reduce(dA, y, s["mean"], s["invstd"], dgamma, dbeta, coef, ws)
        first = s["x_img"] is not None
        if head is not None:
            assert dA is None and fused_stats and not first
            dY = self._new(B, H, W, C)
            ops.conv1x1_head_bn_apply(head[0], y, head[1], s["mean"], s["invstd"], coef, dY)
        elif pool is not None:
            assert dA is None and fused_stats and not first
            dY = self._new(B, H, W, C)
            ops.maxpool_bwd_apply(pool[0], pool[1], y, s["mean"], s["invstd"], coef, dY, dSkip2=pool[2])
        else:
            dY = Act(dA.buf, dA.coff, dA.C)
            if not first:
                ops.bn_bwd_apply(dA, y, s["mean"], s["invstd"], coef, dY)
        grads[s["pbn"] + "weight"] = dgamma
        grads[s["pbn"] + "bias"] = dbeta
        gb = self._gbuf(s["pconv"] + "bias", sd[s["pconv"] + "bias"])
        self._zero_pending.append(gb)
        grads[s["pconv"] + "bias"] = gb
        dW = self._gbuf(s["pconv"] + "weight", w)
        if s["x_img"] is not None:
            wsb = self.scratch.get("wg", self.lib.cmu_conv3x3_c1_wgrad_ws_bytes(B, H, W, C))
            same_w = (_C1W_RECOMP and s.get("w_ver") == (w._version, w.data_ptr(), ops.PARAM_GENERATION)
                      and getattr(self.lib, "cmu_conv3x3_c1_wgrad_bn_w", None) is not None)
            ops.conv3x3_c1_wgrad_bn(s["x_img"], dA, y, y.scale, y.shift, s["mean"], s["invstd"], coef, dW, wsb, s["mask"], s["mps"],
                                    w=w.detach() if same_w else None)
        else:
            Cin = w.shape[1]
            wsb = self.scratch.get("wg", self.lib.cmu_conv3x3_wgrad_ws_bytes(B, H, W, Cin, C, self.dt))
            ops.conv3x3_wgrad(s["x"], dY, dW, wsb)
        grads[s["pconv"] + "weight"] = dW
        if not need_dx or first:
            return None
        dX = dx_out if dx_out is not None else self._new(B, H, W, w.shape[1])
        if next_bn is not None and next_bn["y"].C == dX.C and (_FUSE_DGRAD_BN == "1" or (_FUSE_DGRAD_BN == "64" and dX.C <= 64)
                                                                or (_FUSE_DGRAD_BN == "128" and dX.C <= 128)):
            slab = self._tile_slab(next_bn["y"])
            ops.conv3x3_dgrad_bn(dY, self._wp(s["pconv"], w, True), dX, next_bn["y"], next_bn["mean"], next_bn["invstd"], slab)
            next_bn["bstats"] = slab
        else:
            ops.conv3x3_fwd(dY, self._wp(s["pconv"], w, True), dX, None)
        return dX

    @staticmethod
    def n_down(sd, prefix=""):
        n = 0
        while f"{prefix}down_conv{n + 1}.double_conv.double_conv.0.weight" in sd:
            n += 1
        return n

    def encoder_forward(self, sd, x_bhw, training, prefix="", mask=None, mask_per_sample=False, skip_out=None, skip_affine=None):
        B, H, W = x_bhw.shape
        nd = self.n_down(sd, prefix)
        assert H % (1 << nd) == 0 and W % (1 << nd) == 0, f"H,W must be multiples of {1 << nd}"
        ctx = {"levels": [], "prefix": prefix}
        self._nbt_defer += 1
        x_act, x_img = None, x_bhw.contiguous()
        h, w_ = H, W
        for i in range(1, nd + 1):
            p = f"{prefix}down_conv{i}.double_conv.double_conv."
            C = sd[p + "0.weight"].shape[0]
            out2 = skip_out[i - 1] if skip_out is not None else self._new(B, h, w_, C)
            s1, s2 = self._double_conv_fwd(sd, p, x_act, out2, training, x_img, mask if i == 1 else None, mask_per_sample,
                                           affine_out2=skip_affine[i - 1] if skip_affine is not None else None)
            pooled = self._new(B, h // 2, w_ // 2, C)
            ops.bnrelu_maxpool_fwd(s2["y"], pooled)
            ctx["levels"].append({"s1": s1, "s2": s2, "pooled": pooled})
            x_act, x_img = pooled, None
            h, w_ = h // 2, w_ // 2
        p = f"{prefix}double_conv.double_conv."
        C = sd[p + "0.weight"].shape[0]
        s1, s2 = self._double_conv_fwd(sd, p, x_act, self._new(B, h, w_, C), training, x_img, mask if nd == 0 else None, mask_per_sample)
        ctx["bott"] = {"s1": s1, "s2": s2}
        ctx["latent"] = s2["y"]
        ctx["skips"] = [lv["s2"]["y"] for lv in ctx["levels"]]
        self._nbt_defer -= 1
        self.flush_counters()
        return ctx

    def encoder_backward(self, sd, ctx, d_latent, d_skips, grads, after_bottleneck=None):
        b = ctx["bott"]
        dA = self._convbn_bwd(sd, b["s2"], d_latent, grads, True, next_bn=b["s1"])
        dP = self._convbn_bwd(sd, b["s1"], dA, grads, len(ctx["levels"]) > 0)
        if after_bottleneck is not None:
            self.flush_zero_bias()
            after_bottleneck()
        for i in range(len(ctx["levels"]), 0, -1):
            lv = ctx["levels"][i - 1]
            y2 = lv["s2"]["y"]
            ds = d_skips[i - 1] if d_skips is not None else None
            ds, ds2 = ds if isinstance(ds, (tuple, list)) else (ds, None)
            if _FUSE_POOL and (ds2 is None or _FUSE_POOL2):
                ops.maxpool_bwd(dP, ds, y2, None, lv["s2"]["mean"], lv["s2"]["invstd"], self._bn_ws(y2.C), dSkip2=ds2)
                dA1 = self._convbn_bwd(sd, lv["s2"], None, grads, True, fused_stats=True, next_bn=lv["s1"], pool=(dP, ds, ds2))
            else:
                dA2 = self._new(y2.B, y2.H, y2.W, y2.C)
                ops.maxpool_bwd(dP, ds, y2, dA2, lv["s2"]["mean"], lv["s2"]["invstd"], self._bn_ws(y2.C), dSkip2=ds2)
                dA1 = self._convbn_bwd(sd, lv["s2"], dA2, grads, True, fused_stats=True, next_bn=lv["s1"])
            dP = self._convbn_bwd(sd, lv["s1"], dA1, grads, i > 1)
        self.flush_zero_bias()
        return None

    def decoder_alloc(self, sd, B, H, W, prefix=""):
        cats = []
        i = 1
        h, w_ = H, W
        while f"{prefix}up_conv{i}.double_conv.double_conv.0.weight" in sd:
            wt = sd[f"{prefix}up_conv{i}.double_conv.double_conv.0.weight"]
            Cout, C2 = wt.shape[0], wt.shape[1]
            Cs = C2 - Cout if f"{prefix}up_conv{i}.up_sample.weight" not in sd else sd[f"{prefix}up_conv{i}.up_sample.weight"].shape[1]
            buf = self._new(B, h, w_, C2).buf
            scale = torch.ones(C2, dtype=torch.float32, device=self.device)
            shift = torch.zeros(C2, dtype=torch.float32, device=self.device)
            cats.append({"buf": buf, "scale": scale, "shift": shift, "Cup": Cs, "Cskip": C2 - Cs})
            i += 1
            h, w_ = h // 2, w_ // 2
        return cats

    def decoder_alloc_shared(self, sd, B, H, W, prefix_a, prefix_b):
        ca, cb = [], []
        i = 1
        h, w_ = H, W
        while f"{prefix_a}up_conv{i}.double_conv.double_conv.0.weight" in sd:
            wa = sd[f"{prefix_a}up_conv{i}.double_conv.double_conv.0.weight"]
            wb = sd.get(f"{prefix_b}up_conv{i}.double_conv.double_conv.0.weight")
            ka, kb = f"{prefix_a}up_conv{i}.up_sample.weight", f"{prefix_b}up_conv{i}.up_sample.weight"
            if wb is None or ka not in sd or kb not in sd:
                return None
            Cup_a, Cup_b = sd[ka].shape[1], sd[kb].shape[1]
            Cs = wa.shape[1] - Cup_a
            epc = 16 // torch.empty(0, dtype=self.tdt).element_size()
            if Cs <= 0 or wb.shape[1] - Cup_b != Cs or any(c % epc for c in (Cup_a, Cup_b, Cs)):
# ... 62 lines not shown
            s_lo = 0 if sf else Cup
            if not (sk.buf is cat["buf"] and sk.coff == sk_off):
                cat["buf"][..., sk_off:sk_off + Cs].copy_(sk.buf[..., sk.coff:sk.coff + sk.C])
            if sk.scale is not None:
                if sk.scale.data_ptr() != cat["scale"][s_lo:].data_ptr():
                    cat["scale"][s_lo:s_lo + Cs].copy_(sk.scale)
                    cat["shift"][s_lo:s_lo + Cs].copy_(sk.shift)
                cat["ident"] = False
                relu_from = -Cs if sf else Cup
            else:
                if not cat.get("ident", False):
                    cat["scale"][s_lo:s_lo + Cs].fill_(1.0)
                    cat["shift"][s_lo:s_lo + Cs].zero_()
                    cat["ident"] = True
                relu_from = Cup + Cs
            wt = sd[p + "up_sample.weight"]
            left = Act(cat["buf"], up_off, Cup)
            ops.convT2x2_fwd(x, self._wpT(p + "up_sample.", wt, 0), sd[p + "up_sample.bias"].detach(), left)
            cat_act = Act(cat["buf"], base, Cup + Cs, cat["scale"], cat["shift"], relu_from)
            Cout = sd[p + "double_conv.double_conv.0.weight"].shape[0]
            s1, s2 = self._double_conv_fwd(sd, p + "double_conv.double_conv.", cat_act, self._new(B, sk.H, sk.W, Cout), training)
            ctx["levels"][i - 1] = {"s1": s1, "s2": s2, "x_up": x, "cat": cat}
            x = s2["y"]
        ctx["out"] = x
        if head:
            K = sd[prefix + "conv_last.weight"].shape[0]
            logits = self._f32(B, K, x.H, x.W)
            ops.conv1x1_head_fwd(x, sd[prefix + "conv_last.weight"].detach().reshape(K, -1), sd[prefix + "conv_last.bias"].detach(), logits)
            ctx["logits"] = logits
        self._nbt_defer -= 1
        self.flush_counters()
        return ctx

    def decoder_backward(self, sd, ctx, dlogits, grads, need_input_grads=True, latent_bn=None):
        prefix = ctx["prefix"]
        x = ctx["out"]
        K = sd[prefix + "conv_last.weight"].shape[0]
        wl = sd[prefix + "conv_last.weight"]
        dWl, dbl = self._gbuf(prefix + "conv_last.weight", wl), self._gbuf(prefix + "conv_last.bias", sd[prefix + "conv_last.bias"])
        ws = self.scratch.get("head", self.lib.cmu_conv1x1_head_bwd_ws_bytes(x.B, x.H, x.W, x.C, K))
        last = ctx["levels"][0]["s2"] if ctx["levels"] else None
        fused = last is not None and last["y"] is x
        dl, wl2 = dlogits.contiguous(), wl.detach().reshape(K, -1)
        head = (dl, wl2) if (fused and _FUSE_HEAD) else None
        dA = None if head is not None else self._new(x.B, x.H, x.W, x.C)
        ops.conv1x1_head_bwd(dl, x, wl2, dA, dWl.view(K, -1), dbl, ws,
                             last["mean"] if fused else None, last["invstd"] if fused else None, self._bn_ws(x.C) if fused else None)
        grads[prefix + "conv_last.weight"] = dWl
        grads[prefix + "conv_last.bias"] = dbl
        nup = len(ctx["levels"])
        d_skips = [None] * nup
        for i in range(1, nup + 1):
            lv = ctx["levels"][i - 1]
            p = f"{prefix}up_conv{i}."
            cat = lv["cat"]
            Cup, Cs = cat["Cup"], cat["Cskip"]
            dA1 = self._convbn_bwd(sd, lv["s2"], dA, grads, True, fused_stats=(fused and i == 1), next_bn=lv["s1"],
                                   head=head if i == 1 else None)
            dcat = self._convbn_bwd(sd, lv["s1"], dA1, grads, True)
            sf = bool(cat.get("skip_first", False))
            d_skips[i - 1] = Act(dcat.buf, 0 if sf else Cup, Cs)
            dleft = Act(dcat.buf, Cs if sf else 0, Cup)
            wt = sd[p + "up_sample.weight"]
            xu = lv["x_up"]
            dWt, dbt = self._gbuf(p + "up_sample.weight", wt), self._gbuf(p + "up_sample.bias", sd[p + "up_sample.bias"])
            wsb = self.scratch.get("wg", self.lib.cmu_convT2x2_wgrad_ws_bytes(xu.B, xu.H, xu.W, xu.C, Cup, self.dt))
            ops.convT2x2_wgrad(xu, dleft, dWt, dbt, wsb)
            grads[p + "up_sample.weight"] = dWt
            grads[p + "up_sample.bias"] = dbt
            if i < nup or need_input_grads:
                dA = self._new(xu.B, xu.H, xu.W, xu.C)
                tgt = ctx["levels"][i]["s2"] if i < nup else latent_bn
                if tgt is not None and tgt["y"].buf is xu.buf and tgt["y"].coff == xu.coff and tgt["y"].C == xu.C:
                    slab = self._tile_slab(tgt["y"])
                    ops.convT2x2_dgrad_bn(dleft, self._wpT(p + "up_sample.", wt, 1), dA, tgt["y"], tgt["mean"], tgt["invstd"], slab)
                    tgt["bstats"] = slab
                else:
                    ops.convT2x2_dgrad(dleft, self._wpT(p + "up_sample.", wt, 1), dA)
            else:
                dA = None
        self.flush_zero_bias()
        return dA, d_skips

    def unet_forward(self, sd, x_bhw, training, mask=None, mask_per_sample=False):
        B, H, W = x_bhw.shape
        key = (B, H, W, self.tdt)
        if self._cats_busy and (self._cats_owner is None or self._cats_owner() is None):
            self._cats_busy = False
        owns = False
        if self._cats_busy:
            cats = self.decoder_alloc(sd, B, H, W, "")
        else:
            if self._cats is None or self._cats[0] != key:
                self._cats = (key, self.decoder_alloc(sd, B, H, W, ""))
            cats = self._cats[1]
            self._cats_busy = bool(training)
            owns = True
        skip_out = [Act(c["buf"], c["Cup"], c["Cskip"]) for c in cats]
        skip_affine = [(c["scale"][c["Cup"]:], c["shift"][c["Cup"]:]) for c in cats]
        ectx = self.encoder_forward(sd, x_bhw, training, "", mask, mask_per_sample, skip_out, skip_affine)
        dctx = self.decoder_forward(sd, ectx["latent"], ectx["skips"], training, "", cats, True)
        ctx = _Ctx(enc=ectx, dec=dctx)
        if owns and training:
            self._cats_owner = weakref.ref(ctx)
        return dctx["logits"], ctx

    def unet_backward(self, sd, ctx, dlogits, after_decoder=None, after_bottleneck=None):
        grads = {}
        d_latent, d_skips = self.decoder_backward(sd, ctx["dec"], dlogits, grads, True, latent_bn=ctx["enc"]["bott"]["s2"])
        if after_decoder is not None:
            after_decoder()
        self.encoder_backward(sd, ctx["enc"], d_latent, d_skips, grads, after_bottleneck)
        if self._cats is not None and ctx["dec"]["cats"] is self._cats[1]:
            self._cats_busy = False
        return grads
```

### cmunet_amd/ops.py

```python
import ctypes
import os

import torch

from . import _lib
from ._lib import F32, F16, BF16, call

TORCH_DT = {F32: torch.float32, F16: torch.float16, BF16: torch.bfloat16}
DT_OF = {v: k for k, v in TORCH_DT.items()}
DT_NAME = {F32: "f32", F16: "f16", BF16: "bf16"}
NAME_DT = {"f32": F32, "fp32": F32, "float32": F32, "f16": F16, "fp16": F16, "float16": F16, "bf16": BF16, "bfloat16": BF16}


def dt_code(dt):
    if isinstance(dt, str):
        return NAME_DT[dt]
    if isinstance(dt, torch.dtype):
        return DT_OF[dt]
    return int(dt)


def _stream():
    return _lib.STREAM

# ... 246 lines not shown
             _p(save_mean), _p(save_invstd), _p(coef), _p(_f32c(dW)), B, H, W, dW.shape[0], dA.dt, _p(ws), _stream())
        return
    call("cmu_conv3x3_c1_wgrad_bn", _p(_f32c(x_bhw)), _p(mask), int(mask_per_sample), dA.ptr(), dA.ld, yraw.ptr(), yraw.ld,
         _p(scale), _p(shift), _p(save_mean), _p(save_invstd), _p(coef), _p(_f32c(dW)), B, H, W, dW.shape[0], dA.dt, _p(ws),
         _stream())


def maxpool_bwd(dP, dSkip, y, dA, save_mean=None, save_invstd=None, bn_ws=None, dSkip2=None):
    call("cmu_maxpool_bwd2", dP.ptr(), dP.ld, None if dSkip is None else dSkip.ptr(), 0 if dSkip is None else dSkip.ld,
         None if dSkip2 is None else dSkip2.ptr(), 0 if dSkip2 is None else dSkip2.ld, y.ptr(), y.ld, _p(y.scale), _p(y.shift),
         None if dA is None else dA.ptr(), 0 if dA is None else dA.ld, _p(save_mean), _p(save_invstd), _p(bn_ws),
         y.B, y.H, y.W, y.C, y.dt, _stream())


def maxpool_bwd_apply(dP, dSkip, y, save_mean, save_invstd, coef, dY, dSkip2=None):
    call("cmu_maxpool_bwd_apply", dP.ptr(), dP.ld, None if dSkip is None else dSkip.ptr(), 0 if dSkip is None else dSkip.ld,
         None if dSkip2 is None else dSkip2.ptr(), 0 if dSkip2 is None else dSkip2.ld, y.ptr(), y.ld, _p(y.scale), _p(y.shift),
         _p(save_mean), _p(save_invstd), _p(_f32c(coef)), dY.ptr(), dY.ld, y.B, y.H, y.W, y.C, y.dt, _stream())


def bn_bwd_finalize(bn_ws, count, dgamma, dbeta, coef):
    call("cmu_bn_bwd_finalize", _p(bn_ws), int(count), _p(dgamma), _p(dbeta), _p(coef), coef.shape[1], _stream())


def bn_bwd_finalize_tiles(bstats, count, dgamma, dbeta, coef, ws):
    call("cmu_bn_bwd_finalize_tiles", _p(bstats), bstats.shape[0], int(count), _p(dgamma), _p(dbeta), _p(coef), coef.shape[1], _p(ws),
         _stream())


def conv3x3_dgrad_bn(dY, wpacked_flip, dX, y, save_mean, save_invstd, bstats):
    call("cmu_conv3x3_dgrad_bn", dY.ptr(), dY.ld, _p(wpacked_flip), dX.ptr(), dX.ld, y.ptr(), y.ld, _p(y.scale), _p(y.shift),
         _p(save_mean), _p(save_invstd), _p(bstats), dX.B, dX.H, dX.W, dY.C, dX.C, dX.dt, _stream(),
         work=2.0 * 9 * dY.C * dX.C * dX.B * dX.H * dX.W)


def convT2x2_dgrad_bn(dOut, wpacked_dgrad, dX, y, save_mean, save_invstd, bstats):
    call("cmu_convT2x2_dgrad_bn", dOut.ptr(), dOut.ld, _p(wpacked_dgrad), dX.ptr(), dX.ld, y.ptr(), y.ld, _p(y.scale), _p(y.shift),
         _p(save_mean), _p(save_invstd), _p(bstats), dX.B, dX.H, dX.W, dX.C, dOut.C, dX.dt, _stream(),
         work=2.0 * 4 * dX.C * dOut.C * dX.B * dX.H * dX.W)


def convT2x2_dgrad(dOut, wpacked_dgrad, dX):
    call("cmu_convT2x2_dgrad", dOut.ptr(), dOut.ld, _p(wpacked_dgrad), dX.ptr(), dX.ld, dX.B, dX.H, dX.W, dX.C, dOut.C,
         dX.dt, _stream(), work=2.0 * 4 * dX.C * dOut.C * dX.B * dX.H * dX.W)


def convT2x2_wgrad(x, dOut, dW, dbias, ws):
    Cin, Cout = dW.shape[0], dW.shape[1]
    call("cmu_convT2x2_wgrad", x.ptr(), x.ld, _p(x.scale), _p(x.shift), x.relu_from, dOut.ptr(), dOut.ld, _p(_f32c(dW)),
         _p(_f32c(dbias)), x.B, x.H, x.W, Cin, Cout, x.dt, _p(ws), _stream(), work=2.0 * 4 * Cin * Cout * x.B * x.H * x.W)


def conv1x1_head_bn_apply(dlogits, x, w, save_mean, save_invstd, coef, dY):
    K = w.shape[0]
    call("cmu_conv1x1_head_bn_apply", _p(_f32c(dlogits)), x.ptr(), x.ld, _p(x.scale), _p(x.shift), _p(_f32c(w)), _p(save_mean),
         _p(save_invstd), _p(_f32c(coef)), dY.ptr(), dY.ld, x.B, x.H, x.W, x.C, K, x.dt, _stream())


def conv1x1_head_bwd(dlogits, x, w, dX, dW, dbias, ws, save_mean=None, save_invstd=None, bn_ws=None):
    K = w.shape[0]
    if dX is None:
        call("cmu_conv1x1_head_bwd", _p(_f32c(dlogits)), x.ptr(), x.ld, _p(x.scale), _p(x.shift), _p(_f32c(w)), None, 0,
             _p(_f32c(dW)), _p(_f32c(dbias)), _p(save_mean), _p(save_invstd), _p(bn_ws), x.B, x.H, x.W, x.C, K, x.dt, _p(ws),
             _stream())
        return
    call("cmu_conv1x1_head_bwd", _p(_f32c(dlogits)), x.ptr(), x.ld, _p(x.scale), _p(x.shift), _p(_f32c(w)), dX.ptr(), dX.ld,
# ... 550 lines not shown
```

### include/cmunet_hip.h

```cpp
#ifndef CMUNET_HIP_H
#define CMUNET_HIP_H

#include <stdint.h>

#ifdef __cplusplus
extern "C" {
#endif

typedef enum { CMU_F32 = 0, CMU_F16 = 1, CMU_BF16 = 2 } cmu_dtype;

#define CMU_OK 0
#define CMU_ERR_ARG (-1)
#define CMU_ERR_UNSUPPORTED (-2)
#define CMU_ERR_WORKSPACE (-3)
#define CMU_ERR_LAUNCH (-4)

const char* cmu_last_error(void);
const char* cmu_last_kernel(void);
int cmu_version(void);
int cmu_set_dispatch_override(const char* name, int value);
int cmu_dtype_size(int dt);

int64_t cmu_pack_conv3x3_elems(int Cin, int Cout, int dt, int transpose_flip);
int cmu_pack_conv3x3(const float* w, void* out, int Cin, int Cout, int dt, int transpose_flip, void* stream);
// ... 13 lines not shown

int64_t cmu_bn_finalize_ws_bytes(int C);
int cmu_bn_finalize(const float* stats, int ntiles, int64_t count, const float* conv_bias, const float* gamma,
                    const float* beta, float* running_mean, float* running_var, float momentum, float eps,
                    int training, float* scale, float* shift, float* save_mean, float* save_invstd,
                    int C, void* ws, void* stream);

int cmu_bnrelu_maxpool_fwd(const void* y, int64_t ldy, const float* scale, const float* shift,
                           void* out, int64_t ldo, int B, int H, int W, int C, int dt, void* stream);

int cmu_convT2x2_fwd(const void* x, int64_t ldx, const float* in_scale, const float* in_shift, int relu_from,
                     const void* wpacked, const float* bias, void* out, int64_t ldo,
                     int B, int H, int W, int Cin, int Cout, int dt, void* stream);

int cmu_conv1x1_head_fwd(const void* x, int64_t ldx, const float* in_scale, const float* in_shift,
                         const float* w , const float* bias, float* logits,
                         int B, int H, int W, int C, int K, int dt, void* stream);

int cmu_apply_to_nchw(const void* y, int64_t ldy, const float* scale, const float* shift, int relu_from,
                      float* out, int B, int H, int W, int C, int dt, void* stream);
int cmu_nchw_to_nhwc(const float* x, void* out, int64_t ldo, int B, int H, int W, int C, int dt, void* stream);
int cmu_nhwc_to_nchw(const void* x, int64_t ldx, float* out, int B, int H, int W, int C, int dt, void* stream);

int64_t cmu_bn_bwd_ws_bytes(int C);
int cmu_bn_bwd_reduce(const void* dA, int64_t ldd, const void* y, int64_t ldy, const float* scale, const float* shift,
                      const float* save_mean, const float* save_invstd, float* dgamma, float* dbeta, float* coef,
                      int B, int H, int W, int C, int dt, void* ws, void* stream);
int cmu_bn_bwd_finalize(const void* bn_ws, int64_t count, float* dgamma, float* dbeta, float* coef, int C, void* stream);
int cmu_bn_bwd_finalize_tiles(const float* bstats, int ntiles, int64_t count, float* dgamma, float* dbeta, float* coef, int C,
                              void* ws, void* stream);
int cmu_conv3x3_dgrad_bn(const void* dY, int64_t ldd, const void* wpacked_flip, void* dX, int64_t ldx, const void* yraw, int64_t ldy,
                         const float* scale, const float* shift, const float* save_mean, const float* save_invstd, float* bstats,
                         int B, int H, int W, int K, int N, int dt, void* stream);
int cmu_bn_bwd_apply(const void* dA, int64_t ldd, const void* y, int64_t ldy, const float* scale, const float* shift,
                     const float* save_mean, const float* save_invstd, const float* coef, void* dY, int64_t ldo,
                     int B, int H, int W, int C, int dt, void* stream);

int64_t cmu_conv3x3_wgrad_ws_bytes(int B, int H, int W, int Cin, int Cout, int dt);
int cmu_conv3x3_wgrad(const void* x, int64_t ldx, const float* in_scale, const float* in_shift, int relu_from,
                      const void* dY, int64_t ldd, float* dW, int B, int H, int W, int Cin, int Cout, int dt,
                      void* ws, void* stream);
int64_t cmu_conv3x3_c1_wgrad_ws_bytes(int B, int H, int W, int Cout);
int cmu_conv3x3_c1_wgrad(const float* x, const uint8_t* mask, int mask_per_sample, const void* dY, int64_t ldd,
                         float* dW, int B, int H, int W, int Cout, int dt, void* ws, void* stream);
int cmu_conv3x3_c1_wgrad_bn(const float* x, const uint8_t* mask, int mask_per_sample, const void* dA, int64_t ldd,
                            const void* yraw, int64_t ldy, const float* scale, const float* shift, const float* save_mean,
                            const float* save_invstd, const float* coef, float* dW, int B, int H, int W, int Cout, int dt,
                            void* ws, void* stream);
int cmu_conv3x3_c1_wgrad_bn_w(const float* x, const uint8_t* mask, int mask_per_sample, const void* dA, int64_t ldd,
                              const float* w, const float* scale, const float* shift, const float* save_mean,
                              const float* save_invstd, const float* coef, float* dW, int B, int H, int W, int Cout, int dt,
                              void* ws, void* stream);

int cmu_maxpool_bwd(const void* dP, int64_t ldp, const void* dSkip, int64_t lds, const void* y, int64_t ldy,
                    const float* scale, const float* shift, void* dA, int64_t lda,
                    const float* save_mean, const float* save_invstd, void* bn_ws,
                    int B, int H, int W, int C, int dt, void* stream);
int cmu_maxpool_bwd2(const void* dP, int64_t ldp, const void* dSkip, int64_t lds, const void* dSkip2, int64_t lds2, const void* y,
                     int64_t ldy, const float* scale, const float* shift, void* dA, int64_t lda,
                     const float* save_mean, const float* save_invstd, void* bn_ws,
                     int B, int H, int W, int C, int dt, void* stream);
int cmu_maxpool_bwd_apply(const void* dP, int64_t ldp, const void* dSkip, int64_t lds, const void* dSkip2, int64_t lds2, const void* y,
                          int64_t ldy, const float* scale, const float* shift, const float* save_mean, const float* save_invstd,
                          const float* coef, void* dY, int64_t ldo, int B, int H, int W, int C, int dt, void* stream);

int cmu_bnrelu_maxpool_fwd_masked(const void* y, int64_t ldy, const float* scale, const float* shift, const uint8_t* active, int f,
                                  void* out, int64_t ldo, int B, int H, int W, int C, int dt, void* stream);
int cmu_maxpool_bwd_masked(const void* dP, int64_t ldp, const void* dSkip, int64_t lds, const void* y, int64_t ldy, const float* scale,
                           const float* shift, const uint8_t* active, int f, void* dA, int64_t lda, int B, int H, int W, int C, int dt,
                           void* stream);

int cmu_convT2x2_dgrad(const void* dOut, int64_t ldd, const void* wpacked_dgrad, void* dX, int64_t ldx,
                       int B, int H, int W, int Cin, int Cout, int dt, void* stream);
int cmu_convT2x2_dgrad_bn(const void* dOut, int64_t ldd, const void* wpacked_dgrad, void* dX, int64_t ldx, const void* yraw,
                          int64_t ldy, const float* scale, const float* shift, const float* save_mean, const float* save_invstd,
                          float* bstats, int B, int H, int W, int Cin, int Cout, int dt, void* stream);
int64_t cmu_convT2x2_wgrad_ws_bytes(int B, int H, int W, int Cin, int Cout, int dt);
int cmu_convT2x2_wgrad(const void* x, int64_t ldx, const float* in_scale, const float* in_shift, int relu_from,
                       const void* dOut, int64_t ldd, float* dW, float* dbias,
                       int B, int H, int W, int Cin, int Cout, int dt, void* ws, void* stream);

int64_t cmu_conv1x1_head_bwd_ws_bytes(int B, int H, int W, int C, int K);
int cmu_conv1x1_head_bwd(const float* dlogits, const void* x, int64_t ldx, const float* in_scale, const float* in_shift,
                         const float* w, void* dX, int64_t ldo, float* dW, float* dbias,
                         const float* save_mean, const float* save_invstd, void* bn_ws ,
                         int B, int H, int W, int C, int K, int dt, void* ws, void* stream);
int cmu_conv1x1_head_bn_apply(const float* dlogits, const void* x, int64_t ldx, const float* in_scale, const float* in_shift,
                              const float* w, const float* save_mean, const float* save_invstd, const float* coef, void* dY,
                              int64_t ldo, int B, int H, int W, int C, int K, int dt, void* stream);

int64_t cmu_masked_mse_ws_bytes(int B, int H);
int cmu_masked_mse_fwd_bwd(const float* logits, int K, int channel, const float* img, const uint8_t* mask,
                           float* loss, float* dlogits, float loss_scale, const void* amp_state, int B, int H, int W, void* ws,
                           void* stream);

int64_t cmu_softmax_ce_dice_ws_bytes(int B, int H, int W);
int cmu_softmax_ce_dice_fwd_bwd(const float* logits, const double* y1h, float* out, float* dlogits, float loss_scale,
// ... 224 lines not shown
```

Before: 837.0 images/sec.

## Fold encoder BN backward reductions into decoder dgrad and pooled conv epilogues

Computes the BN-backward channel sums for encoder skip outputs inside the decoder's conv3x3 dgrad epilogue, restricted to the skip channel window, and inside the pooled-layer dgrad. The separate maxpool backward sum pass then only reduces channels whose gamma/beta are ill-conditioned for the fold; all other channels exit early. A new finalize kernel combines the skip slab, the pooled slab and the fallback sums. The goal is to remove a full read pass over large encoder activations, at the cost of extra epilogue work and a numerical-conditioning heuristic.

```diff
diff --git a/cmunet_amd/_lib.py b/cmunet_amd/_lib.py
--- a/cmunet_amd/_lib.py
+++ b/cmunet_amd/_lib.py
@@ -93,6 +93,9 @@
     "cmu_convT2x2_dgrad_bn": (_I, [_P, _L, _P, _P, _L, _P, _L, _P, _P, _P, _P, _P, _I, _I, _I, _I, _I, _I, _P]),
     "cmu_conv3x3_dgrad_bn": (_I, [_P, _L, _P, _P, _L, _P, _L, _P, _P, _P, _P, _P, _I, _I, _I, _I, _I, _I, _P]),
     "cmu_bn_bwd_finalize_tiles": (_I, [_P, _I, _L, _P, _P, _P, _I, _P, _P]),
+    "cmu_conv3x3_dgrad_bn_win": (_I, [_P, _L, _P, _P, _L, _P, _L, _P, _P, _P, _P, _P, _I, _I, _I, _I, _I, _I, _I, _I, _P]),
+    "cmu_maxpool_bwd_sums_fallback": (_I, [_P, _L, _P, _L, _P, _L, _P, _L, _P, _P, _P, _P, _P, _P, _P, _I, _I, _I, _I, _I, _P]),
+    "cmu_bn_bwd_finalize_pool": (_I, [_P, _I, _I, _I, _P, _I, _P, _P, _P, _L, _P, _P, _P, _I, _P, _P]),
     "cmu_convT2x2_wgrad_ws_bytes": (_L, [_I, _I, _I, _I, _I, _I]),
     "cmu_convT2x2_wgrad": (_I, [_P, _L, _P, _P, _I, _P, _L, _P, _P, _I, _I, _I, _I, _I, _I, _P, _P]),
     "cmu_conv1x1_head_bwd_ws_bytes": (_L, [_I, _I, _I, _I, _I]),
diff --git a/cmunet_amd/csrc/backward_elem.hip b/cmunet_amd/csrc/backward_elem.hip
--- a/cmunet_amd/csrc/backward_elem.hip
+++ b/cmunet_amd/csrc/backward_elem.hip
@@ -11,7 +11,6 @@
 #define CMU_POOLA_PPT 0
 #endif
 constexpr int POOLB_MAX_BLOCKS = CMU_POOLB_BLOCKS, HEADB_MAX_BLOCKS = CMU_HEADB_BLOCKS;
-constexpr int BNWS_HDR = 16;
 
 __device__ static inline float sum_over_rows(float v, float* red, int tid, int cpb, int ppb) {
     __syncthreads();
@@ -144,27 +143,7 @@
     const int cl = threadIdx.x & 15, part = threadIdx.x >> 4;
     const int c = blockIdx.x * 16 + cl;
     double s1 = 0.0, s2 = 0.0;
-    if (c < C) {
-        constexpr int U = 8;
-        int b = part;
-        for (; b + 16 * (U - 1) < nblocks; b += 16 * U) {
-            float a[U], q[U];
-#pragma unroll
-            for (int u = 0; u < U; ++u) {
-                a[u] = ws[((int64_t)(b + 16 * u) * 2 + 0) * C + c];
-                q[u] = ws[((int64_t)(b + 16 * u) * 2 + 1) * C + c];
-            }
-#pragma unroll
-            for (int u = 0; u < U; ++u) {
-                s1 += (double)a[u];
-                s2 += (double)q[u];
-            }
-        }
-        for (; b < nblocks; b += 16) {
-            s1 += (double)ws[((int64_t)b * 2 + 0) * C + c];
-            s2 += (double)ws[((int64_t)b * 2 + 1) * C + c];
-        }
-    }
+    if (c < C) cmu_bn_ws_rows(ws, nblocks, C, c, part, s1, s2);
     red[0][part][cl] = s1;
     red[1][part][cl] = s2;
     __syncthreads();
@@ -372,7 +351,8 @@
                                                          int cpb, int ppb, const float* __restrict__ mean,
                                                          const float* __restrict__ invstd, float* __restrict__ bn_ws,
                                                          const float* __restrict__ coef, const uint8_t* __restrict__ amask = nullptr,
-                                                         int mf = 0, int msbits = 0) {
+                                                         int mf = 0, int msbits = 0, const float* __restrict__ fb_gamma = nullptr,
+                                                         const float* __restrict__ fb_beta = nullptr) {
     constexpr int EPC = TR::EPC;
     constexpr int ES = (int)sizeof(typename TR::elem_t);
     __shared__ float red[MODE == 2 ? 1 : FOLD_G * 256];
@@ -380,7 +360,16 @@
     const int nchunk = C / EPC;
     const int ch = blockIdx.y * cpb + tid % cpb;
     const int prow = tid / cpb;
-    const bool active = prow < ppb && ch < nchunk;
+    bool active = prow < ppb && ch < nchunk;
+    if (MODE == 1 && fb_gamma != nullptr) {
+        if (blockIdx.x == 0 && blockIdx.y == 0 && tid == 0) *reinterpret_cast<int*>(bn_ws) = (int)gridDim.x;
+        bool ill = false;
+        if (active)
+#pragma unroll
+            for (int e = 0; e < EPC; ++e) ill |= cmu_pool_fold_illcond(fb_gamma[ch * EPC + e], fb_beta[ch * EPC + e]);
+        active = ill;
+        if (!__syncthreads_or(active ? 1 : 0)) return;
+    }
     const int Ho = H / 2, Wo = W / 2;
     const int64_t npool = (int64_t)B * Ho * Wo;
     float sc[EPC], sh[EPC], mu[EPC], is[EPC], s1[EPC], s2[EPC], c1[EPC], c2[EPC];
@@ -489,7 +478,8 @@
 template <class TR>
 static int maxpool_bwd_t(const void* dP, int64_t ldp, const void* dS, int64_t lds, const void* dS2, int64_t lds2, const void* y, int64_t ldy, const float* scale,
                          const float* shift, void* dA, int64_t lda, int B, int H, int W, int C, const float* mean, const float* invstd,
-                         void* bn_ws, hipStream_t st, const float* coef = nullptr, const uint8_t* amask = nullptr, int mf = 0) {
+                         void* bn_ws, hipStream_t st, const float* coef = nullptr, const uint8_t* amask = nullptr, int mf = 0,
+                         const float* fb_gamma = nullptr, const float* fb_beta = nullptr) {
     int cpb, ppb, gy;
     chunk_geometry(C / TR::EPC, &cpb, &ppb, &gy);
     const int64_t npool = (int64_t)B * (H / 2) * (W / 2);
@@ -502,7 +492,7 @@
 #define CMU_POOLB_LAUNCH(MODE_)                                                                                                            \
     hipLaunchKernelGGL((maxpool_bwd_kernel<TR, MODE_>), dim3(gx, gy), dim3(256), 0, st, (const unsigned char*)dP, ldp, (const unsigned char*)dS, lds, \
                        (const unsigned char*)dS2, lds2, (const unsigned char*)y, ldy, scale, shift, (unsigned char*)dA, lda, B, H, W, C, cpb, ppb, \
-                       mean, invstd, (float*)bn_ws, coef, amask, mf, amask ? sp_shift_bits(H, mf) : 0)
+                       mean, invstd, (float*)bn_ws, coef, amask, mf, amask ? sp_shift_bits(H, mf) : 0, fb_gamma, fb_beta)
     if (coef != nullptr) CMU_POOLB_LAUNCH(2);
     else if (dA == nullptr) CMU_POOLB_LAUNCH(1);
     else CMU_POOLB_LAUNCH(0);
@@ -1069,3 +1059,18 @@
     CMU_DISPATCH_DT(dt, conv3x3_c1_wgrad_t, x, mask, mask_per_sample, dA, ldd, dW, B, H, W, Cout, ws, (hipStream_t)stream, nullptr, 0, scale,
                     shift, save_mean, save_invstd, coef, w);
 }
+
+extern "C" int cmu_maxpool_bwd_sums_fallback(const void* dP, int64_t ldp, const void* dSkip, int64_t lds, const void* dSkip2, int64_t lds2,
+                                             const void* y, int64_t ldy, const float* scale, const float* shift, const float* save_mean,
+                                             const float* save_invstd, const float* gamma, const float* beta, void* bn_ws, int B, int H, int W,
+                                             int C, int dt, void* stream) {
+    CMU_CHECK_ARG(bn_ws && save_mean && save_invstd && gamma && beta && scale && shift, "cmu_maxpool_bwd_sums_fallback: null argument");
+    CMU_CHECK_ARG(dSkip2 == nullptr || dSkip != nullptr, "cmu_maxpool_bwd_sums_fallback: dSkip2 without dSkip");
+    int rc;
+    if ((rc = check_pair("cmu_maxpool_bwd_sums_fallback(dP,y)", dP, ldp, y, ldy, C, dt))) return rc;
+    if (dSkip && (rc = check_pair("cmu_maxpool_bwd_sums_fallback(dSkip,y)", dSkip, lds, y, ldy, C, dt))) return rc;
+    if (dSkip2 && (rc = check_pair("cmu_maxpool_bwd_sums_fallback(dSkip2,y)", dSkip2, lds2, y, ldy, C, dt))) return rc;
+    CMU_CHECK_ARG(B > 0 && H > 0 && W > 0 && H % 2 == 0 && W % 2 == 0, "cmu_maxpool_bwd_sums_fallback: bad dims (%d,%d)", H, W);
+    CMU_DISPATCH_DT(dt, maxpool_bwd_t, dP, ldp, dSkip, lds, dSkip2, lds2, y, ldy, scale, shift, nullptr, 0, B, H, W, C, save_mean, save_invstd,
+                    bn_ws, (hipStream_t)stream, nullptr, nullptr, 0, gamma, beta);
+}
diff --git a/cmunet_amd/csrc/common.h b/cmunet_amd/csrc/common.h
--- a/cmunet_amd/csrc/common.h
+++ b/cmunet_amd/csrc/common.h
@@ -235,3 +235,29 @@
     }
     out[0] = c0; out[1] = c1; out[2] = c2; out[3] = c3;
 }
+
+constexpr int BNWS_HDR = 16;
+__device__ __forceinline__ void cmu_bn_ws_rows(const float* __restrict__ ws, int nblocks, int C, int c, int part, double& s1, double& s2) {
+    constexpr int U = 8;
+    int b = part;
+    for (; b + 16 * (U - 1) < nblocks; b += 16 * U) {
+        float a[U], q[U];
+#pragma unroll
+        for (int u = 0; u < U; ++u) {
+            a[u] = ws[((int64_t)(b + 16 * u) * 2 + 0) * C + c];
+            q[u] = ws[((int64_t)(b + 16 * u) * 2 + 1) * C + c];
+        }
+#pragma unroll
+        for (int u = 0; u < U; ++u) {
+            s1 += (double)a[u];
+            s2 += (double)q[u];
+        }
+    }
+    for (; b < nblocks; b += 16) {
+        s1 += (double)ws[((int64_t)b * 2 + 0) * C + c];
+        s2 += (double)ws[((int64_t)b * 2 + 1) * C + c];
+    }
+}
+__device__ __forceinline__ bool cmu_pool_fold_illcond(float gamma, float beta) {
+    return !(fabsf(beta) <= CMU_POOL_FOLD_T * fabsf(gamma)) || gamma == 0.f;
+}
diff --git a/cmunet_amd/csrc/conv_igemm.hip b/cmunet_amd/csrc/conv_igemm.hip
--- a/cmunet_amd/csrc/conv_igemm.hip
+++ b/cmunet_amd/csrc/conv_igemm.hip
@@ -27,11 +27,20 @@
     int64_t ldbx;
     const float *b_scale, *b_shift, *b_mean, *b_invstd;
     float* bstats;
+    int bw0, bwn;
     int buf_ok;
     unsigned fd_nblk[2], fd_tx[2], fd_ty[2];
     const int* tile_list;
     const int* tile_count;
 };
+__device__ __forceinline__ bool ig_bwin(const IGParams& p, int nw, int& col, int64_t& ldbx) {
+    const int c = nw - p.bw0;
+    const bool in = (unsigned)c < (unsigned)p.bwn;
+    col = in ? c : 0;
+    ldbx = in ? p.ldbx : 0;
+    return in;
+}
+
 static inline void cmu_fastdiv_init(unsigned d, unsigned* out) {
     unsigned s = 0;
     while ((1ull << s) < d) ++s;
@@ -361,16 +370,18 @@
     }
     constexpr int CPRp = C::BN / C::EPC;
     u32x4 xr[CPRp];
-    if ((MODE != MODE_CONVT_FWD) && p.bstats != nullptr) {
+    int bcol = 0;
+    int64_t bld = 0;
+    const bool bs = (MODE != MODE_CONVT_FWD) && p.bstats != nullptr && ig_bwin(p, n0, bcol, bld);
+    if (bs) {
 #pragma unroll
         for (int it = 0; it < CPRp; ++it) {
             const int idx = it * 64 + lane;
             const int m = idx / CPRp, q = idx % CPRp;
             const int row = 4 * wave + 2 * (m >> 5) + pm_row(m & 31), col = pm_col(m & 31);
             const int gy = ty0 + row < p.H ? ty0 + row : p.H - 1, gx = tx0 + col < p.W ? tx0 + col : p.W - 1;
-            int n = n0 + q * C::EPC;
-            n = n < p.N ? n : 0;
-            const int64_t xo = (((int64_t)b * p.H + gy) * p.W + gx) * p.ldbx + n;
+            const int n = n0 + q * C::EPC < p.N ? bcol + q * C::EPC : 0;
+            const int64_t xo = (((int64_t)b * p.H + gy) * p.W + gx) * bld + n;
             xr[it] = ld_global16(reinterpret_cast<const unsigned char*>(p.bx) + xo * (int64_t)sizeof(elem_t));
         }
     }
@@ -407,14 +418,13 @@
     }
     constexpr int CPR = C::BN / C::EPC;
     unsigned char* yb = reinterpret_cast<unsigned char*>(p.y);
-    const bool bs = (MODE != MODE_CONVT_FWD) && p.bstats != nullptr;
     constexpr int EPCc = C::EPC;
     float bsc[EPCc], bsh[EPCc], bmu[EPCc], bis[EPCc], bs1[EPCc], bs2[EPCc];
     const int nq = n0 + (lane % CPR) * EPCc;
     if (bs) {
 #pragma unroll
         for (int e = 0; e < EPCc; ++e) {
-            const int c = nq + e < p.N ? nq + e : 0;
+            const int c = nq + e < p.N ? bcol + (nq - n0) + e : 0;
             bsc[e] = p.b_scale[c]; bsh[e] = p.b_shift[c]; bmu[e] = p.b_mean[c]; bis[e] = p.b_invstd[c];
             bs1[e] = bs2[e] = 0.f;
         }
@@ -471,8 +481,8 @@
                 a += stat_lds[(w4 * C::BN + tid) * 2 + 0];
                 q += stat_lds[(w4 * C::BN + tid) * 2 + 1];
             }
-            p.bstats[(tile * 2 + 0) * p.N + n0 + tid] = a;
-            p.bstats[(tile * 2 + 1) * p.N + n0 + tid] = q;
+            p.bstats[(tile * 2 + 0) * p.bwn + bcol + tid] = a;
+            p.bstats[(tile * 2 + 1) * p.bwn + bcol + tid] = q;
         }
     }
 }
@@ -882,23 +892,41 @@
     return CMU_OK;
 }
 
-extern "C" int cmu_conv3x3_dgrad_bn(const void* dY, int64_t ldd, const void* wpacked_flip, void* dX, int64_t ldx, const void* yraw,
-                                    int64_t ldy, const float* scale, const float* shift, const float* save_mean,
-                                    const float* save_invstd, float* bstats, int B, int H, int W, int K, int N, int dt, void* stream) {
-    CMU_CHECK_ARG(B > 0 && H > 0 && W > 0 && K > 0 && N > 0, "cmu_conv3x3_dgrad_bn: bad dims");
-    CMU_CHECK_ARG(cmu_dtype_size(dt) > 0, "cmu_conv3x3_dgrad_bn: bad dtype %d", dt);
+static int conv3x3_dgrad_bn_any(const char* name, const void* dY, int64_t ldd, const void* wpacked_flip, void* dX, int64_t ldx, const void* yraw,
+                                int64_t ldy, const float* scale, const float* shift, const float* save_mean, const float* save_invstd, float* bstats,
+                                int B, int H, int W, int K, int N, int win0, int nwin, int dt, void* stream) {
+    CMU_CHECK_ARG(B > 0 && H > 0 && W > 0 && K > 0 && N > 0, "%s: bad dims", name);
+    CMU_CHECK_ARG(cmu_dtype_size(dt) > 0, "%s: bad dtype %d", name, dt);
     int rc;
     if ((rc = check_act("cmu_conv3x3_dgrad_bn(dY)", dY, ldd, K, dt))) return rc;
     if ((rc = check_act("cmu_conv3x3_dgrad_bn(dX)", dX, ldx, N, dt))) return rc;
-    if ((rc = check_bnstats("cmu_conv3x3_dgrad_bn(yraw)", yraw, ldy, scale, shift, save_mean, save_invstd, bstats, N, dt))) return rc;
-    CMU_CHECK_ARG(wpacked_flip && cmu_aligned16(wpacked_flip), "cmu_conv3x3_dgrad_bn: packed weights null/unaligned");
-    CMU_CHECK_ARG((int64_t)B * cmu_div_up(H, CMU_TH) * cmu_div_up(W, CMU_TW) * cmu_div_up(N, 64) < (1ll << 31), "cmu_conv3x3_dgrad_bn: grid too large");
+    if ((rc = check_bnstats("cmu_conv3x3_dgrad_bn(yraw)", yraw, ldy, scale, shift, save_mean, save_invstd, bstats, nwin, dt))) return rc;
+    CMU_CHECK_ARG(wpacked_flip && cmu_aligned16(wpacked_flip), "%s: packed weights null/unaligned", name);
+    CMU_CHECK_ARG((int64_t)B * cmu_div_up(H, CMU_TH) * cmu_div_up(W, CMU_TW) * cmu_div_up(N, 64) < (1ll << 31), "%s: grid too large", name);
     IGParams p = {};
     p.x = dY; p.ldx = ldd; p.w = wpacked_flip; p.y = dX; p.ldy = ldx;
     p.B = B; p.H = H; p.W = W; p.K = K; p.N = N; p.Cq = N;
     p.bx = yraw; p.ldbx = ldy; p.b_scale = scale; p.b_shift = shift; p.b_mean = save_mean; p.b_invstd = save_invstd; p.bstats = bstats;
+    p.bw0 = win0; p.bwn = nwin;
     fill_tiles(p);
     CMU_DISPATCH_DT(dt, conv3x3_fwd_t, p, (hipStream_t)stream);
+}
+
+extern "C" int cmu_conv3x3_dgrad_bn(const void* dY, int64_t ldd, const void* wpacked_flip, void* dX, int64_t ldx, const void* yraw,
+                                    int64_t ldy, const float* scale, const float* shift, const float* save_mean,
+                                    const float* save_invstd, float* bstats, int B, int H, int W, int K, int N, int dt, void* stream) {
+    return conv3x3_dgrad_bn_any("cmu_conv3x3_dgrad_bn", dY, ldd, wpacked_flip, dX, ldx, yraw, ldy, scale, shift, save_mean, save_invstd, bstats,
+                                B, H, W, K, N, 0, N, dt, stream);
+}
+
+extern "C" int cmu_conv3x3_dgrad_bn_win(const void* dY, int64_t ldd, const void* wpacked_flip, void* dX, int64_t ldx, const void* yraw,
+                                        int64_t ldy, const float* scale, const float* shift, const float* save_mean,
+                                        const float* save_invstd, float* bstats, int B, int H, int W, int K, int N, int win0, int nwin, int dt,
+                                        void* stream) {
+    CMU_CHECK_ARG(win0 >= 0 && nwin > 0 && win0 % 64 == 0 && nwin % 64 == 0 && win0 + nwin <= N,
+                  "cmu_conv3x3_dgrad_bn_win: window [%d, %d + %d) must be whole 64-channel blocks inside N=%d", win0, win0, nwin, N);
+    return conv3x3_dgrad_bn_any("cmu_conv3x3_dgrad_bn_win", dY, ldd, wpacked_flip, dX, ldx, yraw, ldy, scale, shift, save_mean, save_invstd,
+                                bstats, B, H, W, K, N, win0, nwin, dt, stream);
 }
 
 extern "C" int cmu_convT2x2_dgrad_bn(const void* dOut, int64_t ldd, const void* wpacked_dgrad, void* dX, int64_t ldx, const void* yraw,
@@ -916,6 +944,7 @@
     p.x = dOut; p.ldx = ldd; p.w = wpacked_dgrad; p.y = dX; p.ldy = ldx;
     p.B = B; p.H = H; p.W = W; p.K = Cout; p.N = Cin; p.Cq = Cout;
     p.bx = yraw; p.ldbx = ldy; p.b_scale = scale; p.b_shift = shift; p.b_mean = save_mean; p.b_invstd = save_invstd; p.bstats = bstats;
+    p.bw0 = 0; p.bwn = Cin;
     fill_tiles(p);
     CMU_DISPATCH_DT(dt, convT_dgrad_t, p, (hipStream_t)stream);
 }
diff --git a/cmunet_amd/csrc/conv_igemm3.inc b/cmunet_amd/csrc/conv_igemm3.inc
--- a/cmunet_amd/csrc/conv_igemm3.inc
+++ b/cmunet_amd/csrc/conv_igemm3.inc
@@ -150,11 +150,12 @@
     unsigned char* my = smem + wave * C::EPI_WAVE;
     unsigned char* yb = reinterpret_cast<unsigned char*>(p.y);
     constexpr int CPR = C::NFP * 32 / EPC;
-    auto write_slab = [&](float* dst) {
+    auto write_slab = [&](float* dst, int off, int ld) {
         if (tid < TWB * NB) {
             const int half = tid / NB, c = tid % NB;
             const int tx16 = TWB * tx + half, tiles16 = (p.W + 15) / 16;
-            if (tx16 < tiles16 && n0 + c < p.N) {
+            const int col = n0 + c - off;
+            if (tx16 < tiles16 && n0 + c < p.N && (unsigned)col < (unsigned)ld) {
                 float a = 0.f, q = 0.f;
 #pragma unroll
                 for (int wr = 0; wr < C::RB; ++wr) {
@@ -163,8 +164,8 @@
                     q += stat_lds[(wv * 64 + (c & 63)) * 2 + 1];
                 }
                 const int64_t t16 = ((int64_t)b * p.tilesY + ty) * tiles16 + tx16;
-                dst[(t16 * 2 + 0) * p.N + n0 + c] = a;
-                dst[(t16 * 2 + 1) * p.N + n0 + c] = q;
+                dst[(t16 * 2 + 0) * ld + col] = a;
+                dst[(t16 * 2 + 1) * ld + col] = q;
             }
         }
     };
@@ -179,6 +180,9 @@
 #pragma unroll
         for (int j = 0; j < 2; ++j) badd[j] = p.bias[cq64 ? co_w + 32 * j + r : (nw + 32 * j + r) % p.Cq];
     }
+    int bcol = 0;
+    int64_t bld = 0;
+    if (p.bstats != nullptr) ig_bwin(p, n0 + wn * 64, bcol, bld);
 #pragma unroll
     for (int jp = 0; jp < 2 / C::NFP; ++jp) {
         if (jp > 0) __syncthreads();
@@ -190,9 +194,9 @@
                 const int m = idx / CPR, q = idx % CPR;
                 const int row = row0 + 2 * (m >> 5) + pm_row(m & 31), col = col0 + pm_col(m & 31);
                 const int gy = ty0 + row < p.H ? ty0 + row : p.H - 1, gx = tx0 + col < p.W ? tx0 + col : p.W - 1;
-                const int n = n0 + wn * 64 + jp * C::NFP * 32 + q * EPC;
+                const int n = bcol + jp * C::NFP * 32 + q * EPC;
                 const int64_t pixel = ((int64_t)b * p.H + gy) * p.W + gx;
-                xr[it] = ld_global16(reinterpret_cast<const unsigned char*>(p.bx) + (pixel * p.ldbx + n) * (int64_t)sizeof(elem_t));
+                xr[it] = ld_global16(reinterpret_cast<const unsigned char*>(p.bx) + (pixel * bld + n) * (int64_t)sizeof(elem_t));
             }
         }
 #pragma unroll
@@ -206,11 +210,11 @@
                         TR::from_float(acc[i][jp * C::NFP + jj][e] + badd[jp * C::NFP + jj]);
                 }
         __syncthreads();
-        if (jp == 0 && p.stats != nullptr) write_slab(p.stats);
+        if (jp == 0 && p.stats != nullptr) write_slab(p.stats, 0, p.N);
         float bsc[EPC], bsh[EPC], bs1[EPC], bs2[EPC];
         const int nq = n0 + wn * 64 + jp * C::NFP * 32 + (lane % CPR) * EPC;
         if (p.bstats != nullptr) {
-            ig3_bst_consts<EPC>(p.b_scale, p.b_shift, nq, bsc, bsh);
+            ig3_bst_consts<EPC>(p.b_scale, p.b_shift, bcol + (nq - n0 - wn * 64), bsc, bsh);
 #pragma unroll
             for (int e = 0; e < EPC; ++e) bs1[e] = bs2[e] = 0.f;
         }
@@ -235,13 +239,13 @@
             }
         }
         if (p.bstats != nullptr) {
-            const int nb0 = n0 + wn * 64 + jp * C::NFP * 32;
+            const int nb0 = bcol + jp * C::NFP * 32;
             ig3_bst_fold<EPC>(bs1, bs2, lane, p.b_mean + nb0, p.b_invstd + nb0, stat_lds + (wave * 64 + jp * C::NFP * 32) * 2);
         }
     }
     if (p.bstats != nullptr) {
         __syncthreads();
-        write_slab(p.bstats);
+        write_slab(p.bstats, p.bw0, p.bwn);
     }
 }
 
diff --git a/cmunet_amd/csrc/conv_igemm3p.inc b/cmunet_amd/csrc/conv_igemm3p.inc
--- a/cmunet_amd/csrc/conv_igemm3p.inc
+++ b/cmunet_amd/csrc/conv_igemm3p.inc
@@ -294,21 +294,25 @@
         const int q = lane % CPR;
         const int64_t pix0 = ((int64_t)t.b * p.H + ty0 + row0) * p.W + tx0 + col0;
         const int cl = (lane >> 3) & 3;
+        int bcol = 0;
+        int64_t bld = 0;
+        if (BST) ig_bwin(p, t.n0 + wn * 64, bcol, bld);
         unsigned yoff[2], xoff[2];
 #pragma unroll
         for (int c = 0; c < 2; ++c) {
             yoff[c] = (unsigned)((((h ^ c) * p.W + cl) * p.ldy + q * EPC) * C::ES);
-            xoff[c] = BST ? (unsigned)((((h ^ c) * p.W + cl) * p.ldbx + q * EPC) * C::ES) : 0u;
+            xoff[c] = BST ? (unsigned)((((h ^ c) * p.W + cl) * bld + q * EPC) * C::ES) : 0u;
         }
 #pragma unroll
         for (int jp = 0; jp < 2 / C::NFP; ++jp) {
             const int n = t.n0 + wn * 64 + jp * C::NFP * 32 + q * EPC;
             const int nw = t.n0 + wn * 64 + jp * C::NFP * 32;
             unsigned char* ybase = yb + (pix0 * p.ldy + nw) * (int64_t)C::ES;
-            const unsigned char* xbase = reinterpret_cast<const unsigned char*>(p.bx) + (pix0 * p.ldbx + nw) * (int64_t)C::ES;
+            const int bw = bcol + jp * C::NFP * 32;
+            const unsigned char* xbase = reinterpret_cast<const unsigned char*>(p.bx) + (pix0 * bld + bw) * (int64_t)C::ES;
             float bsc[EPC], bsh[EPC], bs1[EPC], bs2[EPC];
             if (BST) {
-                ig3_bst_consts<EPC>(p.b_scale, p.b_shift, n, bsc, bsh);
+                ig3_bst_consts<EPC>(p.b_scale, p.b_shift, bw + q * EPC, bsc, bsh);
 #pragma unroll
                 for (int e = 0; e < EPC; ++e) bs1[e] = bs2[e] = 0.f;
             }
@@ -316,14 +320,14 @@
 #pragma unroll
                 for (int it = 0; it < NIT; ++it) {
                     if (FULL) {
-                        const int soff = ((2 * (u >> 1)) * p.W + 4 * (2 * (u & 1) + it)) * (int)p.ldbx * C::ES;
+                        const int soff = ((2 * (u >> 1)) * p.W + 4 * (2 * (u & 1) + it)) * (int)bld * C::ES;
                         xr[it] = ld_global16(xbase + soff + xoff[(it ^ u) & 1]);
                     } else {
                         const int m = 16 * (u & 1) + (it * 64 + lane) / CPR;
                         const int row = row0 + 2 * (u >> 1) + pm_row(m), col = col0 + pm_col(m);
                         const int gy = ty0 + row < p.H ? ty0 + row : p.H - 1, gx = tx0 + col < p.W ? tx0 + col : p.W - 1;
                         const int64_t pixel = ((int64_t)t.b * p.H + gy) * p.W + gx;
-                        xr[it] = ld_global16(reinterpret_cast<const unsigned char*>(p.bx) + (pixel * p.ldbx + n) * (int64_t)sizeof(elem_t));
+                        xr[it] = ld_global16(reinterpret_cast<const unsigned char*>(p.bx) + (pixel * bld + bw + q * EPC) * (int64_t)sizeof(elem_t));
                     }
                 }
             };
@@ -387,7 +391,7 @@
             }
             IG3P_STAMP_E(6);
             __builtin_amdgcn_wave_barrier();
-            if (BST) ig3_bst_fold<EPC>(bs1, bs2, lane, p.b_mean + nw, p.b_invstd + nw, stat_lds + (wave * 64 + jp * C::NFP * 32) * 2);
+            if (BST) ig3_bst_fold<EPC>(bs1, bs2, lane, p.b_mean + bw, p.b_invstd + bw, stat_lds + (wave * 64 + jp * C::NFP * 32) * 2);
         }
     };
     auto epilogue = [&](const Item t) { epilogue_impl(t, std::integral_constant<bool, !PART>{}); };
@@ -399,7 +403,8 @@
             const int blk = tid / NB, c = tid % NB;
             const int vhalf = blk / TWB, half = blk % TWB;
             const int tx16 = TWB * t.tx + half, tiles16 = (p.W + 15) / 16;
-            if (tx16 < tiles16 && t.n0 + c < p.N) {
+            const int col = BST ? t.n0 + c - p.bw0 : t.n0 + c, ld = BST ? p.bwn : p.N;
+            if (tx16 < tiles16 && t.n0 + c < p.N && (unsigned)col < (unsigned)ld) {
                 float a = 0.f, q2 = 0.f;
 #pragma unroll
                 for (int wr = 0; wr < C::RB / THB; ++wr) {
@@ -408,8 +413,8 @@
                     q2 += stat_lds[(wv * 64 + (c & 63)) * 2 + 1];
                 }
                 const int64_t t16 = ((int64_t)t.b * (THB * p.tilesY) + THB * t.ty + vhalf) * tiles16 + tx16;
-                dst[(t16 * 2 + 0) * p.N + t.n0 + c] = a;
-                dst[(t16 * 2 + 1) * p.N + t.n0 + c] = q2;
+                dst[(t16 * 2 + 0) * ld + col] = a;
+                dst[(t16 * 2 + 1) * ld + col] = q2;
             }
         }
     };
diff --git a/cmunet_amd/csrc/conv_igemm5.inc b/cmunet_amd/csrc/conv_igemm5.inc
--- a/cmunet_amd/csrc/conv_igemm5.inc
+++ b/cmunet_amd/csrc/conv_igemm5.inc
@@ -436,13 +436,16 @@
             IG5_STAMP(2);
 #endif
         } else {
-            const unsigned char* xbase = reinterpret_cast<const unsigned char*>(p.bx) + (pix0 * p.ldbx + nw) * (int64_t)C::ES;
-            const unsigned xoff = (unsigned)((pi * (int)p.ldbx + 8 * g) * C::ES);
-            const int64_t xrow = (int64_t)p.W * p.ldbx * C::ES;
+            int bcol;
+            int64_t bld;
+            ig_bwin(p, nw, bcol, bld);
+            const unsigned char* xbase = reinterpret_cast<const unsigned char*>(p.bx) + (pix0 * bld + bcol) * (int64_t)C::ES;
+            const unsigned xoff = (unsigned)((pi * (int)bld + 8 * g) * C::ES);
+            const int64_t xrow = (int64_t)p.W * bld * C::ES;
             float bsc[2][EPC], bsh[2][EPC], bs1[2][EPC], bs2[2][EPC];
 #pragma unroll
             for (int s = 0; s < 2; ++s) {
-                ig3_bst_consts<EPC>(p.b_scale, p.b_shift, nw + 32 * s + 8 * g, bsc[s], bsh[s]);
+                ig3_bst_consts<EPC>(p.b_scale, p.b_shift, bcol + 32 * s + 8 * g, bsc[s], bsh[s]);
 #pragma unroll
                 for (int e = 0; e < EPC; ++e) bs1[s][e] = bs2[s][e] = 0.f;
             }
@@ -499,9 +502,10 @@
         float* dst = BST ? p.bstats : p.stats;
         int tl = threadIdx.x;
         asm volatile("" : "+v"(tl));
-        if (dst != nullptr && tl < 2 * C::NB) {
+        const int half = tl / C::NB, c = tl % C::NB;
+        const int col = BST ? t.n0 + c - p.bw0 : t.n0 + c, ld = BST ? p.bwn : p.N;
+        if (dst != nullptr && tl < 2 * C::NB && (unsigned)col < (unsigned)ld) {
             const float* stat_lds = reinterpret_cast<const float*>(smem + C::STAT_OFF + par * C::STAT_PAR);
-            const int half = tl / C::NB, c = tl % C::NB;
             const int tx16 = 2 * t.tx + half, tiles16 = p.W / 16;
             float a = 0.f, q2 = 0.f;
 #pragma unroll
@@ -510,10 +514,10 @@
                 a += stat_lds[(wv * 64 + (c & 63)) * 2 + 0];
                 q2 += stat_lds[(wv * 64 + (c & 63)) * 2 + 1];
             }
-            if (BST) q2 = (q2 - p.b_mean[t.n0 + c] * a) * p.b_invstd[t.n0 + c];
+            if (BST) q2 = (q2 - p.b_mean[col] * a) * p.b_invstd[col];
             const int64_t t16 = ((int64_t)t.b * p.tilesY + t.ty) * tiles16 + tx16;
-            dst[(t16 * 2 + 0) * p.N + t.n0 + c] = a;
-            dst[(t16 * 2 + 1) * p.N + t.n0 + c] = q2;
+            dst[(t16 * 2 + 0) * ld + col] = a;
+            dst[(t16 * 2 + 1) * ld + col] = q2;
         }
     };
 
@@ -564,15 +568,18 @@
             if constexpr (BST) {
                 const Item t = decode(i_mma);
                 const int64_t pix0 = ((int64_t)t.b * p.H + t.ty * C::TH + 8 * wrow) * p.W + t.tx * C::TW + 16 * wcol;
-                const uint64_t xa = reinterpret_cast<uint64_t>(p.bx) + (uint64_t)((pix0 * p.ldbx + t.n0 + wn * 64) * (int64_t)C::ES);
+                int bcol;
+                int64_t bld;
+                ig_bwin(p, t.n0 + wn * 64, bcol, bld);
+                const uint64_t xa = reinterpret_cast<uint64_t>(p.bx) + (uint64_t)((pix0 * bld + bcol) * (int64_t)C::ES);
                 typedef __attribute__((ext_vector_type(4))) int i32x4_t;
                 const i32x4_t xd = {__builtin_amdgcn_readfirstlane((int)(uint32_t)xa), __builtin_amdgcn_readfirstlane((int)((xa >> 32) & 0xffffu)), -1, 0x00020000};
                 int ln = tid & 63;
                 asm volatile("" : "+v"(ln));
                 const int n16l = ln & 15, gl = ln >> 4;
                 const int pil = n16l < 4 ? n16l : (n16l < 12 ? n16l + 4 : n16l - 8);
-                const unsigned xoffl = (unsigned)((pil * (int)p.ldbx + 8 * gl) * C::ES);
-                const unsigned xrowl = (unsigned)((int64_t)p.W * p.ldbx * C::ES);
+                const unsigned xoffl = (unsigned)((pil * (int)bld + 8 * gl) * C::ES);
+                const unsigned xrowl = (unsigned)((int64_t)p.W * bld * C::ES);
                 const unsigned lds0 = (unsigned)(C::BX_OFF + wave * C::BX_WAVE);
 #pragma unroll
                 for (int i = 0; i < 4; ++i)
@@ -669,6 +676,9 @@
     return CMU_OK;
 }
 
+#ifndef CMU_V5_MIN_K_BSTW_DEFAULT
+#define CMU_V5_MIN_K_BSTW_DEFAULT 128
+#endif
 template <class TR>
 static bool igemm5_eligible(const IGParams& p) {
     if constexpr (sizeof(typename TR::elem_t) != 2) return false;
@@ -678,7 +688,9 @@
     if (p.N % 128 != 0 || p.K % 64 != 0) return false;
     static const int min_k = []() { const char* e = getenv("CMU_V5_MIN_K"); return e ? atoi(e) : 128; }();
     static const int min_k_bst = []() { const char* e = getenv("CMU_V5_MIN_K_BST"); return e ? atoi(e) : 256; }();
-    if (p.K < min_k || (p.bstats != nullptr && p.K < min_k_bst)) return false;
+    static const int min_k_bstw = []() { const char* e = getenv("CMU_V5_MIN_K_BSTW"); return e ? atoi(e) : CMU_V5_MIN_K_BSTW_DEFAULT; }();
+    const bool windowed = p.bstats != nullptr && p.bwn < p.N;
+    if (p.K < min_k || (p.bstats != nullptr && p.K < (windowed ? min_k_bstw : min_k_bst))) return false;
     if (p.H % 16 != 0 || p.W % 32 != 0) return false;
     if ((int64_t)p.B * (p.H / 16) * (p.W / 32) * (p.N / 128) >= (1ll << 30)) return false;
     return !igemm3_narrow_blocks(p);
diff --git a/cmunet_amd/csrc/elementwise.hip b/cmunet_amd/csrc/elementwise.hip
--- a/cmunet_amd/csrc/elementwise.hip
+++ b/cmunet_amd/csrc/elementwise.hip
@@ -378,6 +378,103 @@
     return CMU_OK;
 }
 
+struct PoolFoldSlabs {
+    const float* s[2];
+    int ntiles[2], ld[2], off[2], nsplit[2];
+};
+__global__ void bn_reduce_slab2_kernel(PoolFoldSlabs q, int C, double* __restrict__ ws) {
+    __shared__ double red[2][4][64];
+    const int z = blockIdx.z;
+    const float* __restrict__ stats = q.s[z];
+    const int nsplit = q.nsplit[z], split = blockIdx.y;
+    if (stats == nullptr || split >= nsplit) return;
+    const int c = blockIdx.x * 64 + (threadIdx.x & 63);
+    const int part = threadIdx.x >> 6;
+    const int ntiles = q.ntiles[z], ld = q.ld[z], off = q.off[z];
+    const int per = (ntiles + nsplit - 1) / nsplit;
+    const int t0 = split * per, t1 = min(ntiles, t0 + per);
+    double s1 = 0.0, s2 = 0.0;
+    if (c < C)
+        for (int t = t0 + part; t < t1; t += 4) {
+            s1 += (double)stats[((int64_t)t * 2 + 0) * ld + off + c];
+            s2 += (double)stats[((int64_t)t * 2 + 1) * ld + off + c];
+        }
+    red[0][part][threadIdx.x & 63] = s1;
+    red[1][part][threadIdx.x & 63] = s2;
+    __syncthreads();
+    if (part == 0 && c < C) {
+        const int l = threadIdx.x;
+        double* w = ws + (int64_t)z * BN_MAX_SPLITS * 2 * C;
+        w[((int64_t)split * 2 + 0) * C + c] = red[0][0][l] + red[0][1][l] + red[0][2][l] + red[0][3][l];
+        w[((int64_t)split * 2 + 1) * C + c] = red[1][0][l] + red[1][1][l] + red[1][2][l] + red[1][3][l];
+    }
+}
+__global__ void bn_bwd_final_pool_kernel(const double* __restrict__ ws, int nsk, int nsp, const float* __restrict__ fb,
+                                         const float* __restrict__ gamma, const float* __restrict__ beta, double count, float* dgamma,
+                                         float* dbeta, float* coef, int C) {
+    __shared__ double red[4][16][16];
+    const int cl = threadIdx.x & 15, part = threadIdx.x >> 4;
+    const int c = blockIdx.x * 16 + cl;
+    const double* __restrict__ wk = ws;
+    const double* __restrict__ wp = ws + (int64_t)BN_MAX_SPLITS * 2 * C;
+    double a1 = 0.0, a2 = 0.0, b1 = 0.0, b2 = 0.0;
+    bool ill = false;
+    float g = 1.f, be = 0.f;
+    if (c < C) {
+        g = gamma[c];
+        be = beta[c];
+        ill = cmu_pool_fold_illcond(g, be);
+        if (ill) {
+            cmu_bn_ws_rows(fb + BNWS_HDR / 4, *reinterpret_cast<const int*>(fb), C, c, part, a1, a2);
+        } else {
+            for (int s = part; s < nsk; s += 16) {
+                a1 += wk[((int64_t)s * 2 + 0) * C + c];
+                a2 += wk[((int64_t)s * 2 + 1) * C + c];
+            }
+            for (int s = part; s < nsp; s += 16) {
+                b1 += wp[((int64_t)s * 2 + 0) * C + c];
+                b2 += wp[((int64_t)s * 2 + 1) * C + c];
+            }
+        }
+    }
+    red[0][part][cl] = a1;
+    red[1][part][cl] = a2;
+    red[2][part][cl] = b1;
+    red[3][part][cl] = b2;
+    __syncthreads();
+    if (part != 0 || c >= C) return;
+    double s1 = 0.0, s2 = 0.0, p1 = 0.0, p2 = 0.0;
+    for (int q = 0; q < 16; ++q) { s1 += red[0][q][cl]; s2 += red[1][q][cl]; }
+    if (!ill) {
+        for (int q = 0; q < 16; ++q) { p1 += red[2][q][cl]; p2 += red[3][q][cl]; }
+        s1 = s1 + p1;
+        s2 = s2 + (p2 - (double)be * p1) / (double)g;
+    }
+    if (dbeta) dbeta[c] = (float)s1;
+    if (dgamma) dgamma[c] = (float)s2;
+    coef[c] = (float)(s1 / count);
+    coef[C + c] = (float)(s2 / count);
+}
+extern "C" int cmu_bn_bwd_finalize_pool(const float* skip, int skip_ntiles, int skip_ld, int skip_off, const float* pool, int pool_ntiles,
+                                        const void* bn_ws, const float* gamma, const float* beta, int64_t count, float* dgamma, float* dbeta,
+                                        float* coef, int C, void* ws, void* stream) {
+    CMU_CHECK_ARG(pool && bn_ws && gamma && beta && coef && ws && C > 0 && pool_ntiles > 0 && count > 0, "cmu_bn_bwd_finalize_pool: bad args");
+    CMU_CHECK_ARG(skip == nullptr || (skip_ntiles > 0 && skip_off >= 0 && skip_ld >= skip_off + C),
+                  "cmu_bn_bwd_finalize_pool: skip slab of %d tiles, row %d, offset %d cannot hold C=%d", skip_ntiles, skip_ld, skip_off, C);
+    hipStream_t st = (hipStream_t)stream;
+    auto splits = [](int ntiles) { int n = ntiles / 16; return n < 1 ? 1 : (n > BN_MAX_SPLITS ? BN_MAX_SPLITS : n); };
+    PoolFoldSlabs q = {};
+    q.s[0] = skip; q.ntiles[0] = skip ? skip_ntiles : 0; q.ld[0] = skip_ld; q.off[0] = skip_off; q.nsplit[0] = skip ? splits(skip_ntiles) : 0;
+    q.s[1] = pool; q.ntiles[1] = pool_ntiles; q.ld[1] = C; q.off[1] = 0; q.nsplit[1] = splits(pool_ntiles);
+    const int gy = q.nsplit[0] > q.nsplit[1] ? q.nsplit[0] : q.nsplit[1];
+    hipLaunchKernelGGL(bn_reduce_slab2_kernel, dim3(cmu_div_up(C, 64), gy, 2), dim3(256), 0, st, q, C, (double*)ws);
+    CMU_CHECK_LAUNCH("cmu_bn_bwd_finalize_pool(reduce)");
+    hipLaunchKernelGGL(bn_bwd_final_pool_kernel, dim3(cmu_div_up(C, 16)), dim3(256), 0, st, (const double*)ws, q.nsplit[0], q.nsplit[1],
+                       (const float*)bn_ws, gamma, beta, (double)count, dgamma, dbeta, coef, C);
+    CMU_CHECK_LAUNCH("cmu_bn_bwd_finalize_pool");
+    return CMU_OK;
+}
+
 #ifndef CMU_C1F_WAVES
 #define CMU_C1F_WAVES 4
 #endif
diff --git a/cmunet_amd/engine.py b/cmunet_amd/engine.py
--- a/cmunet_amd/engine.py
+++ b/cmunet_amd/engine.py
@@ -17,6 +17,8 @@
 _POISON_NEW = os.environ.get("CMU_POISON_NEW", "0") == "1"
 _FUSE_POOL2 = os.environ.get("CMU_POOL_FUSE2", "1") != "0"
 _C1W_RECOMP = os.environ.get("CMU_C1W_RECOMP", "1") != "0"
+_POOL_FOLD = os.environ.get("CMU_POOL_FOLD", "1") != "0"
+_POOL_FOLD_MIN_K = int(os.environ.get("CMU_POOL_FOLD_MIN_K", "256"))
 
 
 class _Scratch:
@@ -169,7 +171,19 @@
         n = ops.ntiles(y.B, y.H, y.W)
         return self.scratch.get("bst", n * 2 * y.C * 4)[:n * 2 * y.C * 4].view(torch.float32).view(n, 2, y.C)
 
-    def _convbn_bwd(self, sd, s, dA, grads, need_dx, dx_out=None, fused_stats=False, next_bn=None, head=None, pool=None):
+    def _ident(self, C):
+        t = self.__dict__.setdefault("_ident_c", {}).get(C)
+        if t is None:
+            t = (torch.ones(C, dtype=torch.float32, device=self.device), torch.zeros(C, dtype=torch.float32, device=self.device))
+            self._ident_c[C] = t
+        return t
+
+    def _pooled_bn(self, pooled):
+        one, zero = self._ident(pooled.C)
+        return {"y": Act(pooled.buf, pooled.coff, pooled.C, one, zero, 0), "mean": zero, "invstd": one}
+
+    def _convbn_bwd(self, sd, s, dA, grads, need_dx, dx_out=None, fused_stats=False, next_bn=None, head=None, pool=None, skip_bn=None,
+                    pool_fold=None):
         y = s["y"]
         B, H, W, C = y.B, y.H, y.W, y.C
         w = sd[s["pconv"] + "weight"]
@@ -180,6 +194,9 @@
         if bst is not None:
             ops.bn_bwd_finalize_tiles(bst, B * H * W, dgamma, dbeta, coef,
                                       self.scratch.get("bnfin", self.lib.cmu_bn_finalize_ws_bytes(C)))
+        elif pool_fold is not None:
+            ops.bn_bwd_finalize_pool(pool_fold[0], 0, pool_fold[1], ws, sd[s["pbn"] + "weight"].detach(), sd[s["pbn"] + "bias"].detach(),
+                                     B * H * W, dgamma, dbeta, coef, self.scratch.get("bnfinp", 2 * self.lib.cmu_bn_finalize_ws_bytes(C)))
         elif fused_stats:
             ops.bn_bwd_finalize(ws, B * H * W, dgamma, dbeta, coef)
         else:
@@ -217,7 +234,14 @@
         if not need_dx or first:
             return None
         dX = dx_out if dx_out is not None else self._new(B, H, W, w.shape[1])
-        if next_bn is not None and next_bn["y"].C == dX.C and (_FUSE_DGRAD_BN == "1" or (_FUSE_DGRAD_BN == "64" and dX.C <= 64)
+        if skip_bn is not None:
+            ys, win0 = skip_bn
+            ny = ys["y"]
+            n = ops.ntiles(B, H, W)
+            slab = self.scratch.get(("skipbst", H, W, ny.C), n * 2 * ny.C * 4)[:n * 2 * ny.C * 4].view(torch.float32).view(n, 2, ny.C)
+            ops.conv3x3_dgrad_bn_win(dY, self._wp(s["pconv"], w, True), dX, ny, ys["mean"], ys["invstd"], slab, win0)
+            ys["skip_bstats"] = slab
+        elif next_bn is not None and next_bn["y"].C == dX.C and (_FUSE_DGRAD_BN == "1" or (_FUSE_DGRAD_BN == "64" and dX.C <= 64)
                                                                 or (_FUSE_DGRAD_BN == "128" and dX.C <= 128)):
             slab = self._tile_slab(next_bn["y"])
             ops.conv3x3_dgrad_bn(dY, self._wp(s["pconv"], w, True), dX, next_bn["y"], next_bn["mean"], next_bn["invstd"], slab)
@@ -263,25 +287,40 @@
         return ctx
 
     def encoder_backward(self, sd, ctx, d_latent, d_skips, grads, after_bottleneck=None):
+        levels = ctx["levels"]
+        dsk = []
+        for i in range(1, len(levels) + 1):
+            ds = d_skips[i - 1] if d_skips is not None else None
+            dsk.append(ds if isinstance(ds, (tuple, list)) else (ds, None))
+        fold = [_POOL_FOLD and _FUSE_POOL and dsk[i][0] is not None and dsk[i][1] is None and "skip_bstats" in levels[i]["s2"]
+                for i in range(len(levels))]
+        skip_slabs = [lv["s2"].pop("skip_bstats", None) for lv in levels]
         b = ctx["bott"]
         dA = self._convbn_bwd(sd, b["s2"], d_latent, grads, True, next_bn=b["s1"])
-        dP = self._convbn_bwd(sd, b["s1"], dA, grads, len(ctx["levels"]) > 0)
+        pooled_bn = self._pooled_bn(levels[-1]["pooled"]) if levels and fold[-1] else None
+        dP = self._convbn_bwd(sd, b["s1"], dA, grads, len(levels) > 0, next_bn=pooled_bn)
         if after_bottleneck is not None:
             self.flush_zero_bias()
             after_bottleneck()
-        for i in range(len(ctx["levels"]), 0, -1):
-            lv = ctx["levels"][i - 1]
+        for i in range(len(levels), 0, -1):
+            lv = levels[i - 1]
             y2 = lv["s2"]["y"]
-            ds = d_skips[i - 1] if d_skips is not None else None
-            ds, ds2 = ds if isinstance(ds, (tuple, list)) else (ds, None)
-            if _FUSE_POOL and (ds2 is None or _FUSE_POOL2):
+            ds, ds2 = dsk[i - 1]
+            pslab = pooled_bn.pop("bstats", None) if pooled_bn is not None else None
+            if fold[i - 1] and pslab is not None:
+                g2, b2 = sd[lv["s2"]["pbn"] + "weight"].detach(), sd[lv["s2"]["pbn"] + "bias"].detach()
+                ops.maxpool_bwd_sums_fallback(dP, ds, y2, lv["s2"]["mean"], lv["s2"]["invstd"], g2, b2, self._bn_ws(y2.C))
+                dA1 = self._convbn_bwd(sd, lv["s2"], None, grads, True, fused_stats=True, next_bn=lv["s1"], pool=(dP, ds, None),
+                                       pool_fold=(skip_slabs[i - 1], pslab))
+            elif _FUSE_POOL and (ds2 is None or _FUSE_POOL2):
                 ops.maxpool_bwd(dP, ds, y2, None, lv["s2"]["mean"], lv["s2"]["invstd"], self._bn_ws(y2.C), dSkip2=ds2)
                 dA1 = self._convbn_bwd(sd, lv["s2"], None, grads, True, fused_stats=True, next_bn=lv["s1"], pool=(dP, ds, ds2))
             else:
                 dA2 = self._new(y2.B, y2.H, y2.W, y2.C)
                 ops.maxpool_bwd(dP, ds, y2, dA2, lv["s2"]["mean"], lv["s2"]["invstd"], self._bn_ws(y2.C), dSkip2=ds2)
                 dA1 = self._convbn_bwd(sd, lv["s2"], dA2, grads, True, fused_stats=True, next_bn=lv["s1"])
-            dP = self._convbn_bwd(sd, lv["s1"], dA1, grads, i > 1)
+            pooled_bn = self._pooled_bn(levels[i - 2]["pooled"]) if i > 1 and fold[i - 2] else None
+            dP = self._convbn_bwd(sd, lv["s1"], dA1, grads, i > 1, next_bn=pooled_bn)
         self.flush_zero_bias()
         return None
 
@@ -410,7 +449,7 @@
         self.flush_counters()
         return ctx
 
-    def decoder_backward(self, sd, ctx, dlogits, grads, need_input_grads=True, latent_bn=None):
+    def decoder_backward(self, sd, ctx, dlogits, grads, need_input_grads=True, latent_bn=None, skip_bn=None):
         prefix = ctx["prefix"]
         x = ctx["out"]
         K = sd[prefix + "conv_last.weight"].shape[0]
@@ -435,7 +474,9 @@
             Cup, Cs = cat["Cup"], cat["Cskip"]
             dA1 = self._convbn_bwd(sd, lv["s2"], dA, grads, True, fused_stats=(fused and i == 1), next_bn=lv["s1"],
                                    head=head if i == 1 else None)
-            dcat = self._convbn_bwd(sd, lv["s1"], dA1, grads, True)
+            K1 = sd[p + "double_conv.double_conv.0.weight"].shape[0]
+            dcat = self._convbn_bwd(sd, lv["s1"], dA1, grads, True,
+                                    skip_bn=self._skip_window(cat, skip_bn[i - 1] if skip_bn and K1 >= _POOL_FOLD_MIN_K else None))
             sf = bool(cat.get("skip_first", False))
             d_skips[i - 1] = Act(dcat.buf, 0 if sf else Cup, Cs)
             dleft = Act(dcat.buf, Cs if sf else 0, Cup)
@@ -460,6 +501,15 @@
         self.flush_zero_bias()
         return dA, d_skips
 
+    @staticmethod
+    def _skip_window(cat, ys):
+        if ys is None or not (_POOL_FOLD and _FUSE_POOL) or cat.get("skip_first", False):
+            return None
+        y, Cup, Cs = ys["y"], cat["Cup"], cat["Cskip"]
+        if not (y.buf is cat["buf"] and y.coff == cat.get("base", 0) + Cup and y.C == Cs and y.scale is not None):
+            return None
+        return (ys, Cup) if Cup % 64 == 0 and Cs % 64 == 0 else None
+
     def unet_forward(self, sd, x_bhw, training, mask=None, mask_per_sample=False):
         B, H, W = x_bhw.shape
         key = (B, H, W, self.tdt)
@@ -485,7 +535,8 @@
 
     def unet_backward(self, sd, ctx, dlogits, after_decoder=None, after_bottleneck=None):
         grads = {}
-        d_latent, d_skips = self.decoder_backward(sd, ctx["dec"], dlogits, grads, True, latent_bn=ctx["enc"]["bott"]["s2"])
+        d_latent, d_skips = self.decoder_backward(sd, ctx["dec"], dlogits, grads, True, latent_bn=ctx["enc"]["bott"]["s2"],
+                                                  skip_bn=[lv["s2"] for lv in ctx["enc"]["levels"]])
         if after_decoder is not None:
             after_decoder()
         self.encoder_backward(sd, ctx["enc"], d_latent, d_skips, grads, after_bottleneck)
diff --git a/cmunet_amd/ops.py b/cmunet_amd/ops.py
--- a/cmunet_amd/ops.py
+++ b/cmunet_amd/ops.py
@@ -302,6 +302,25 @@
     call("cmu_conv3x3_dgrad_bn", dY.ptr(), dY.ld, _p(wpacked_flip), dX.ptr(), dX.ld, y.ptr(), y.ld, _p(y.scale), _p(y.shift),
          _p(save_mean), _p(save_invstd), _p(bstats), dX.B, dX.H, dX.W, dY.C, dX.C, dX.dt, _stream(),
          work=2.0 * 9 * dY.C * dX.C * dX.B * dX.H * dX.W)
+
+
+def conv3x3_dgrad_bn_win(dY, wpacked_flip, dX, y, save_mean, save_invstd, bstats, win0):
+    call("cmu_conv3x3_dgrad_bn_win", dY.ptr(), dY.ld, _p(wpacked_flip), dX.ptr(), dX.ld, y.ptr(), y.ld, _p(y.scale), _p(y.shift),
+         _p(save_mean), _p(save_invstd), _p(bstats), dX.B, dX.H, dX.W, dY.C, dX.C, int(win0), y.C, dX.dt, _stream(),
+         work=2.0 * 9 * dY.C * dX.C * dX.B * dX.H * dX.W)
+
+
+def maxpool_bwd_sums_fallback(dP, dSkip, y, save_mean, save_invstd, gamma, beta, bn_ws, dSkip2=None):
+    call("cmu_maxpool_bwd_sums_fallback", dP.ptr(), dP.ld, None if dSkip is None else dSkip.ptr(), 0 if dSkip is None else dSkip.ld,
+         None if dSkip2 is None else dSkip2.ptr(), 0 if dSkip2 is None else dSkip2.ld, y.ptr(), y.ld, _p(y.scale), _p(y.shift),
+         _p(save_mean), _p(save_invstd), _p(_f32c(gamma)), _p(_f32c(beta)), _p(bn_ws), y.B, y.H, y.W, y.C, y.dt, _stream())
+
+
+def bn_bwd_finalize_pool(skip_slab, skip_off, pool_slab, bn_ws, gamma, beta, count, dgamma, dbeta, coef, ws):
+    C = coef.shape[1]
+    call("cmu_bn_bwd_finalize_pool", _p(skip_slab), 0 if skip_slab is None else skip_slab.shape[0],
+         0 if skip_slab is None else skip_slab.shape[2], int(skip_off), _p(pool_slab), pool_slab.shape[0], _p(bn_ws),
+         _p(_f32c(gamma)), _p(_f32c(beta)), int(count), _p(dgamma), _p(dbeta), _p(coef), C, _p(ws), _stream())
 
 
 def convT2x2_dgrad_bn(dOut, wpacked_dgrad, dX, y, save_mean, save_invstd, bstats):
diff --git a/include/cmunet_hip.h b/include/cmunet_hip.h
--- a/include/cmunet_hip.h
+++ b/include/cmunet_hip.h
@@ -69,6 +69,9 @@
 int cmu_conv3x3_dgrad_bn(const void* dY, int64_t ldd, const void* wpacked_flip, void* dX, int64_t ldx, const void* yraw, int64_t ldy,
                          const float* scale, const float* shift, const float* save_mean, const float* save_invstd, float* bstats,
                          int B, int H, int W, int K, int N, int dt, void* stream);
+int cmu_conv3x3_dgrad_bn_win(const void* dY, int64_t ldd, const void* wpacked_flip, void* dX, int64_t ldx, const void* yraw, int64_t ldy,
+                             const float* scale, const float* shift, const float* save_mean, const float* save_invstd, float* bstats,
+                             int B, int H, int W, int K, int N, int win0, int nwin, int dt, void* stream);
 int cmu_bn_bwd_apply(const void* dA, int64_t ldd, const void* y, int64_t ldy, const float* scale, const float* shift,
                      const float* save_mean, const float* save_invstd, const float* coef, void* dY, int64_t ldo,
                      int B, int H, int W, int C, int dt, void* stream);
@@ -100,6 +103,14 @@
 int cmu_maxpool_bwd_apply(const void* dP, int64_t ldp, const void* dSkip, int64_t lds, const void* dSkip2, int64_t lds2, const void* y,
                           int64_t ldy, const float* scale, const float* shift, const float* save_mean, const float* save_invstd,
                           const float* coef, void* dY, int64_t ldo, int B, int H, int W, int C, int dt, void* stream);
+#define CMU_POOL_FOLD_T 8.0f
+int cmu_maxpool_bwd_sums_fallback(const void* dP, int64_t ldp, const void* dSkip, int64_t lds, const void* dSkip2, int64_t lds2,
+                                  const void* y, int64_t ldy, const float* scale, const float* shift, const float* save_mean,
+                                  const float* save_invstd, const float* gamma, const float* beta, void* bn_ws, int B, int H, int W,
+                                  int C, int dt, void* stream);
+int cmu_bn_bwd_finalize_pool(const float* skip, int skip_ntiles, int skip_ld, int skip_off, const float* pool, int pool_ntiles,
+                             const void* bn_ws, const float* gamma, const float* beta, int64_t count, float* dgamma, float* dbeta,
+                             float* coef, int C, void* ws, void* stream);
 
 int cmu_bnrelu_maxpool_fwd_masked(const void* y, int64_t ldy, const float* scale, const float* shift, const uint8_t* active, int f,
                                   void* out, int64_t ldo, int B, int H, int W, int C, int dt, void* stream);
```

New measurement: 838.6 images/sec (median of 4 runs). Within noise of the previous version (+0.2%).
